# real-stanford/garmentnets

Measured on AMD Instinct MI355X. Metric: garments/s end-to-end predict (PointNet++ -> gridding -> UNet3D -> WNF decode -> marching cubes), higher is better.
Workload: dtype f32 (f16x2 convs, f16x2 decoder MLPs, fp32 accumulation)

## Files before the change

### garmentnets_amd/_lib.py

```python
import ctypes
import os

_HERE = os.path.dirname(os.path.abspath(__file__))
LIB_PATH = os.environ.get("GARMENTNETS_HIP_LIB") or os.path.join(_HERE, "libgarmentnets_hip.so")

GN_OK, GN_EINVAL, GN_ELAUNCH, GN_ECAP = 0, -1, -2, -3

_vp, _i32, _i64, _f32, _f64, _sz = (ctypes.c_void_p, ctypes.c_int, ctypes.c_int64, ctypes.c_float, ctypes.c_double,
                                   ctypes.c_size_t)

PROTOTYPES = {
    "gn_version": [],
    "gn_device_info": [_vp, _vp],
    "gn_segment_ptr": [_vp, _i64, _i32, _vp, _vp],
    "gn_fps": [_vp, _vp, _vp, _vp, _i32, _i32, _vp, _vp],
    "gn_fps_nested": [_vp, _vp, _vp, _vp, _i32, _i32, _vp, _vp, _vp, _vp],
    "gn_fps_workspace_bytes": [_i32, _i32],
    "gn_fps_nested_ws": [_vp, _vp, _vp, _vp, _i32, _i32, _vp, _vp, _vp, _vp, _sz, _vp],
    "gn_ball_query": [_vp, _vp, _vp, _vp, _i32, _i32, _f32, _i32, _vp, _vp, _vp],
    "gn_sa_gather": [_vp, _i32, _i32, _vp, _vp, _vp, _i32, _i32, _i32, _vp, _i32, _vp, _vp],
    "gn_segment_max": [_vp, _i32, _vp, _i32, _i32, _i32, _vp, _i32, _vp],
    "gn_sa_fused_supported": [_i32, _i32, _i32, _i32],
    "gn_sa_fused": [_vp, _i32, _i32, _vp, _vp, _vp, _vp, _i32, _i32, _i32, _vp, _vp, _vp, _vp, _i32, _i32, _i32, _vp, _i32, _vp],
    "gn_sa_fused_scoped": [_vp, _i32, _i32, _vp, _vp, _vp, _vp, _i32, _i32, _i32, _vp, _vp, _vp, _vp, _vp, _i32, _i32, _i32, _vp, _i32, _vp],
    "gn_sa_fused_group": [_vp, _i32, _i32, _vp, _vp, _vp, _vp, _i32, _i32, _i32, _vp, _vp, _vp, _vp, _vp, _i32, _i32, _i32, _vp, _i32, _vp, _i32],
    "gn_sa_fused_auto_group": [_i32, _i32, _i32, _i32, _i32],
    "gn_sa_gather_scoped": [_vp, _i32, _i32, _vp, _vp, _vp, _i32, _i32, _i32, _vp, _vp, _i32, _vp, _vp],
    "gn_global_max_pool": [_vp, _i32, _vp, _i32, _i32, _vp, _i32, _vp],
    "gn_knn_interpolate": [_vp, _i32, _vp, _vp, _vp, _vp, _i32, _i32, _i32, _i32, _vp, _i32, _vp],
    "gn_knn_interpolate_any": [_vp, _i32, _vp, _vp, _vp, _vp, _i32, _i32, _i32, _i32, _vp, _i32, _vp],
    "gn_linear": [_vp, _i32, _vp, _i32, _vp, _vp, _vp, _i32, _i64, _i32, _i32, _vp, _i32, _vp],
    "gn_nocs_head": [_vp, _i32, _i64, _i32, _vp, _vp, _vp, _vp],
    "gn_grid_features": [_vp, _i32, _i32, _vp, _vp, _vp, _vp, _i64, _vp, _vp, _vp, _i32, _i32, _vp, _i32, _vp, _vp],
    "gn_grid_scatter_workspace_bytes": [_i64, _i32, _i32],
    "gn_grid_scatter": [_vp, _i32, _vp, _i64, _i32, _i64, _i32, _vp, _vp, _vp, _sz, _i32, _vp],
    "gn_grid_scatter_ex": [_vp, _i32, _vp, _i64, _i32, _i32, _i64, _i32, _vp, _vp, _vp, _sz, _i32, _vp],
    "gn_channel_stats": [_vp, _i32, _i64, _i32, _vp, _vp, _vp],
    "gn_groupnorm_affine": [_vp, _vp, _i32, _i64, _vp, _vp, _i32, _i64, _i32, _i32, _i32, _f32, _vp, _vp, _vp, _vp, _vp, _vp],
    "gn_channel_stats_any": [_vp, _i32, _i64, _i32, _vp, _vp, _vp],
    "gn_groupnorm_affine_map": [_vp, _vp, _i32, _i32, _i64, _vp, _vp, _i32, _i32, _i64, _i32, _i32, _i32, _f32, _vp, _vp, _vp, _vp, _vp, _vp],
    "gn_conv3d_gcr": [_vp, _i32, _vp, _i32, _vp, _vp, _vp, _i32, _i32, _i32, _i32, _i32, _i32, _vp, _vp, _vp, _vp],
    "gn_conv3d_gcr_split": [_vp, _i32, _vp, _i32, _vp, _vp, _vp, _i32, _vp, _vp, _i32, _i32, _i32, _i32, _i32, _i32, _vp, _vp, _vp, _vp, _vp, _i32, _vp, _vp, _sz, _vp],
    "gn_conv3d_occupancy_workspace_bytes": [_i32, _i32, _i32, _i32],
    "gn_conv_affine_pack_bytes": [_i32, _i32, _i32],
    "gn_conv_affine_pack": [_vp, _i32, _i32, _vp, _vp, _vp, _vp, _i64, _vp, _i32, _vp, _sz, _vp, _vp, _vp, _vp, _vp, _sz, _vp],
    "gn_conv3d_gcr_split_persample": [_vp, _i32, _vp, _vp, _vp, _vp, _vp, _i32, _i32, _i32, _i32, _i32, _i32, _vp, _vp, _vp, _vp, _vp, _i32, _vp, _vp, _sz, _vp],
    "gn_conv_affine_pack_wino_bytes": [_i32, _i32, _i32],
    "gn_conv_affine_pack_wino": [_vp, _i32, _i32, _vp, _vp, _vp, _vp, _i64, _vp, _i32, _vp, _sz, _vp, _vp, _vp, _vp, _vp, _sz, _vp],
    "gn_conv3d_gcr_split_wino": [_vp, _i32, _vp, _vp, _vp, _vp, _vp, _vp, _i32, _i32, _i32, _i32, _i32, _i32, _vp, _vp, _vp, _vp, _vp, _i32, _vp, _sz, _vp],
    "gn_conv3d_gcr_split_wino_partial": [_vp, _i32, _vp, _vp, _vp, _vp, _vp, _vp, _i32, _i32, _i32, _i32, _i32, _i32, _vp, _vp, _vp, _vp, _vp],
    "gn_weight_pack_split_bytes": [_i32, _i32, _i32],
    "gn_weight_pack_split_wino_bytes": [_i32, _i32],
    "gn_weight_pack_upconv_bytes": [_i32, _i32],
    "gn_weight_pack_split": [_vp, _i32, _i32, _i32, _i32, _i32, _vp, _sz, _vp, _vp],
    "gn_weight_pack_split_wino": [_vp, _i32, _i32, _i32, _i32, _vp, _sz, _vp, _vp],
    "gn_weight_pack_upconv": [_vp, _i32, _i32, _i32, _i32, _vp, _sz, _vp, _vp],
    "gn_affine_act": [_vp, _i32, _i64, _i32, _vp, _vp, _vp, _i32, _vp, _vp],
    "gn_upconv_partial": [_vp, _i32, _vp, _vp, _vp, _i32, _vp, _vp, _i32, _i32, _i32, _i32, _i32, _vp, _vp],
    "gn_grid_tile_flags": [_vp, _i64, _i32, _i32, _i32, _i32, _i32, _vp, _vp],
    "gn_maxpool3d_2": [_vp, _i32, _i32, _i32, _i32, _i32, _vp, _vp, _vp, _vp],
    "gn_grid_stats": [_vp, _vp, _i64, _i32, _i64, _i32, _vp, _vp, _vp, _vp],
    "gn_trilinear_sample": [_vp, _i32, _i32, _i32, _i32, _vp, _i32, _i64, _i64, _vp, _i32, _vp],
    "gn_trilinear_sample_batch": [_vp, _i32, _i64, _i32, _i32, _i32, _i32, _vp, _i64, _vp, _i32, _vp],
    "gn_implicit_decode": [_vp, _i32, _i32, _i32, _i32, _vp, _i32, _vp, _i32, _i64, _i64, _vp, _vp, _vp, _vp, _i32, _vp, _vp, _vp, _vp, _i32,
                           _vp, _vp, _vp, _vp, _i32, _vp, _i32, _vp, _vp],
    "gn_ggm3d": [_vp, _i32, _i32, _i32, _f64, _vp, _vp, _vp],
    "gn_minmax": [_vp, _i64, _vp, _vp],
    "gn_ggm3d_batch": [_vp, _i32, _i32, _i32, _i32, _f64, _vp, _vp, _vp],
    "gn_ggm3d_range_workspace_bytes": [_i32, _i32, _i32, _i32],
    "gn_ggm3d_batch_ex": [_vp, _i32, _i32, _i32, _i32, _f64, _vp, _vp, _i32, _vp, _vp, _sz, _vp],
    "gn_minmax_batch": [_vp, _i32, _i64, _vp, _vp],
    "gn_mc33_batch_workspace_bytes": [_i32, _i32, _i32, _i32],
    "gn_mc33_batch": [_vp, _i32, _i32, _i32, _i32, _f64, _vp, _sz, _vp, _vp, _vp, _vp, _i64, _i64, _vp, _vp],
    "gn_mc33_batch_profiled": [_vp, _i32, _i32, _i32, _i32, _f64, _vp, _sz, _vp, _vp, _vp, _vp, _i64, _i64, _vp, _vp, _vp],
    "gn_mc33_workspace_bytes": [_i32, _i32, _i32],
    "gn_mc33": [_vp, _i32, _i32, _i32, _f64, _vp, _sz, _vp, _vp, _vp, _vp, _i64, _i64, _vp, _vp],
    "gn_gather_nn": [_vp, _i32, _i32, _i32, _vp, _i64, _f64, _vp, _vp],
    "gn_gather_nn_batch": [_vp, _i32, _i32, _i32, _i32, _vp, _i64, _f64, _vp, _vp],
    "gn_mesh_compact_workspace_bytes": [_i64, _i64],
    "gn_mesh_largest_component_workspace_bytes": [_i64],
    "gn_mesh_largest_component": [_vp, _i64, _i64, _vp, _sz, _vp, _vp, _vp, _vp],
    "gn_mesh_compact": [_vp, _i32, _vp, _vp, _i64, _i64, _vp, _sz, _vp, _vp, _vp, _vp],
    "gn_scale_verts": [_vp, _i64, _f64, _vp, _vp],
    "gn_implicit_decode_split": [_vp, _i32, _i64, _vp, _vp, _vp, _i32, _i32, _i32, _i32, _vp, _i32, _vp],
    "gn_implicit_decode_split_batch": [_vp, _i32, _i64, _i32, _vp, _vp, _vp, _i32, _i32, _i32, _i32, _vp, _i32, _vp],
    "gn_implicit_decode_batch": [_vp, _i32, _i64, _i32, _i32, _vp, _vp, _vp, _vp, _i32, _vp, _vp, _vp, _vp, _i32, _vp, _vp, _vp, _vp, _i32, _vp, _i32, _vp, _i32, _vp],
    "gn_implicit_decode_lattice_split": [_vp, _i32, _i32, _i32, _i32, _i32, _i64, _i64, _vp, _vp, _vp, _i32, _i32, _i32, _vp, _i32, _vp],
    "gn_decoder_input_scale": [_vp, _i64, _i32, _i32, _f32, _vp, _vp],
    "gn_nearest_neighbor": [_vp, _i64, _vp, _i64, _vp, _vp, _vp],
    "gn_nearest_neighbor_f64_batch": [_vp, _vp, _vp, _i32, _i64, _vp, _vp, _vp],
    "gn_point_mesh_sqdist_batch": [_vp, _vp, _vp, _vp, _i32, _i64, _vp, _vp, _vp, _vp],
    "gn_winding_number_batch": [_vp, _vp, _vp, _vp, _i32, _i64, _vp, _vp, _vp],
    "gn_winding_field_batch": [_vp, _vp, _vp, _i32, _i32, _i32, _i32, _vp, _vp, _vp],
    "gn_distance_field_batch": [_vp, _vp, _vp, _i32, _i32, _i32, _i32, _vp, _vp, _vp, _vp],
    "gn_query_targets_face_chunk": [],
    "gn_query_targets_workspace_bytes": [_i32, _i64, _i64, _i32],
    "gn_query_targets_batch": [_vp, _vp, _vp, _vp, _i32, _i64, _i64, _i32, _i32, _f32, _i32, _vp, _sz, _vp, _vp, _vp, _vp, _vp, _vp],
    "gn_nocs_bin_metrics_workspace_bytes": [_vp, _i32],
    "gn_nocs_bin_metrics": [_vp, _i32, _i32, _i32, _vp, _sz, _vp, _vp],
    "gn_value_losses_workspace_bytes": [_vp, _i32],
    "gn_value_losses": [_vp, _i32, _vp, _sz, _vp, _vp],
    "gn_nocs_bin_loss_bwd": [_vp, _i32, _i32, _i32, _vp, _vp, _vp, _vp],
    "gn_value_losses_bwd": [_vp, _i32, _vp, _vp, _vp],
    "gn_adam_step": [_vp, _i32, _i64, _vp, _i32, _vp],
    "gn_grad_pack": [_vp, _i32, _i64, _vp, _i64, _i32, _vp],
    "gn_grid_scatter_bwd_workspace_bytes": [_i64, _i32, _i64, _i32],
    "gn_grid_scatter_bwd": [_vp, _vp, _vp, _i32, _vp, _i64, _i32, _i32, _i64, _i32, _vp, _sz, _vp, _i32, _vp],
    "gn_segment_max_bwd": [_vp, _i32, _vp, _i32, _vp, _i32, _vp, _i32, _i32, _i32, _vp, _i32, _vp],
    "gn_global_max_pool_bwd": [_vp, _i32, _vp, _i32, _vp, _i32, _vp, _i32, _i32, _vp, _i32, _vp],
    "gn_sa_gather_bwd_workspace_bytes": [_i64, _i64],
    "gn_sa_gather_bwd": [_vp, _i32, _vp, _i64, _i32, _i64, _vp, _sz, _vp, _i32, _vp],
    "gn_knn_neighbours": [_vp, _vp, _vp, _vp, _i32, _i32, _i32, _vp, _vp, _vp],
    "gn_knn_interpolate_bwd_workspace_bytes": [_i64, _i32, _i64],
    "gn_knn_interpolate_bwd": [_vp, _vp, _i32, _i32, _vp, _i32, _i32, _i32, _vp, _sz, _vp, _i32, _vp],
    "gn_trilinear_sample_bwd_workspace_bytes": [_i32, _i64, _i32, _i32, _i32],
    "gn_trilinear_sample_bwd": [_vp, _i32, _vp, _i32, _i32, _i32, _i32, _i32, _vp, _i64, _vp, _sz, _vp, _vp, _vp],
    "gn_conv3d_bwd_weight_workspace_bytes": [_i32, _i32, _i32, _i32, _i32, _i32],
    "gn_conv3d_bwd_weight": [_vp, _i32, _vp, _i32, _vp, _vp, _vp, _vp, _i32, _i32, _i32, _i32, _i32, _vp, _sz, _vp, _vp],
    "gn_relu_mask": [_vp, _vp, _i64, _vp, _vp],
    "gn_relu_mask_max_workspace_bytes": [_i32],
    "gn_relu_mask_max": [_vp, _vp, _i32, _i64, _i32, _vp, _vp, _vp, _vp, _vp, _sz, _vp],
    "gn_conv3d_bwd_weight_split_workspace_bytes": [_i32, _i32, _i32, _i32, _i32, _i32],
    "gn_conv3d_bwd_weight_split": [_vp, _i32, _vp, _i32, _vp, _vp, _vp, _vp, _vp, _vp, _i32, _i32, _i32, _i32, _i32, _vp, _sz, _vp, _vp],
    "gn_groupnorm_bwd_stats_workspace_bytes": [_i32, _i64, _i32],
    "gn_groupnorm_bwd_stats": [_vp, _i32, _i32, _vp, _i32, _i32, _i32, _i32, _i32, _i32, _vp, _sz, _vp, _vp, _vp],
    "gn_groupnorm_bwd_coef": [_vp, _vp, _vp, _vp, _i32, _i32, _i64, _vp, _vp, _vp, _vp, _i32, _i32, _i64, _i32, _i32, _i32, _f32, _vp, _vp, _vp, _vp, _vp,
                              _vp, _vp],
    "gn_groupnorm_bwd_apply": [_vp, _i32, _i32, _vp, _i32, _i32, _i32, _i32, _i32, _i32, _vp, _vp, _vp, _i32, _i32, _i32, _vp, _vp],
    "gn_maxpool3d_2_bwd": [_vp, _vp, _i32, _i32, _i32, _i32, _i32, _vp, _vp],
    "gn_linear_act_bwd_workspace_bytes": [_i64, _i32],
    "gn_linear_act_bwd": [_vp, _i32, _vp, _i32, _vp, _i64, _i32, _vp, _i32, _vp, _sz, _vp, _vp],
    "gn_linear_bwd_weight_workspace_bytes": [_i64, _i32, _i32],
    "gn_linear_bwd_weight": [_vp, _i32, _vp, _i32, _i64, _i32, _i32, _vp, _sz, _vp, _i32, _vp],
    "gn_row_affine": [_vp, _i32, _vp, _vp, _i64, _i32, _vp, _i32, _vp],
    "gn_col_moments_workspace_bytes": [_i64, _i32],
    "gn_col_moments": [_vp, _i32, _i64, _i32, _vp, _sz, _vp, _vp],
    "gn_col_dots_workspace_bytes": [_i64, _i32],
    "gn_col_dots": [_vp, _i32, _vp, _i32, _i64, _i32, _vp, _sz, _vp, _vp],
    "gn_bn_train_bwd_workspace_bytes": [_i64, _i32],
    "gn_bn_train_bwd": [_vp, _i32, _vp, _i32, _vp, _i64, _i32, _vp, _i32, _vp, _sz, _vp, _vp],
    "gn_resident_points": [_vp, _vp, _i32, _i32, _vp, _vp, _vp, _vp, _vp, _vp, _vp, _vp],
    "gn_resident_garment": [_vp, _vp, _i32, _i32, _vp, _vp, _vp, _vp, _vp, _vp, _vp, _vp, _vp, _vp],
    "gn_resident_volume": [_vp, _vp, _i32, _i32, _i32, _vp, _vp, _vp, _vp, _vp, _i32, _vp, _vp, _vp],
    "gn_resident_volume_queries": [_vp, _vp, _i32, _i32, _i32, _vp, _vp, _vp, _vp, _vp, _vp, _vp, _vp],
    "gn_resident_query_targets": [_vp, _vp, _i32, _i64, _i32, _i64, _i64, _i32, _i32, _f32, _i32, _vp, _vp, _sz, _vp, _vp, _vp],
    "gn_resident_surface": [_vp, _vp, _i32, _i32, _vp, _vp, _i32, _vp, _vp, _vp, _vp],
    "gn_resident_mc_surface": [_vp, _vp, _i32, _i32, _vp, _vp, _vp, _vp, _vp],
    "gn_render_points_batch": [_vp, _vp, _vp, _vp, _vp, _i32, _i32, _vp, _vp],
    "gn_color_idx_batch": [_vp, _vp, _vp, _vp, _vp, _i32, _i32, _vp, _vp],
    "gn_render_mesh_batch": [_vp, _vp, _vp, _vp, _vp, _vp, _i32, _i32, _vp, _vp],
    "gn_color_mesh_batch": [_vp, _vp, _vp, _vp, _vp, _vp, _vp, _vp, _i32, _i32, _vp, _vp],
    "gn_depth_render_batch": [_vp, _vp, _vp, _vp, _i32, _vp, _vp, _vp, _i32, _i32, _vp, _vp],
    "gn_depth_cloud_offsets": [_vp, _i32, _i32, _vp, _vp, _vp],
    "gn_depth_cloud_write": [_vp, _vp, _vp, _vp, _vp, _vp, _i32, _vp, _vp, _vp, _vp, _i32, _i32, _i64, _vp, _vp, _vp, _vp],
    "gn_cloth_simulate_batch": [_vp, _vp, _vp, _vp, _vp, _vp, _vp, _vp, _i32, _i64, _i64, _i64, _i32, _vp, _i32, _i32, _vp, _vp],
    "gn_cloth_contact_buckets": [_i32],
    "gn_cloth_contact_workspace_bytes": [_i64, _i32, _i32],
    "gn_cloth_contact_lists": [_vp, _vp, _vp, _i32, _i64, _i32, _i32, _vp, _i32, _i32, _vp, _sz, _vp, _vp, _vp, _vp, _vp, _vp],
    "gn_cloth_simulate_contacts_batch": [_vp, _vp, _vp, _vp, _vp, _vp, _vp, _vp, _i32, _i64, _i64, _i64, _i32, _vp, _i32, _i32, _vp, _vp, _vp, _vp,
                                         _i32, _vp, _vp, _vp, _vp],
}
_RESTYPES = {"gn_weight_pack_split_bytes": _sz, "gn_weight_pack_split_wino_bytes": _sz, "gn_weight_pack_upconv_bytes": _sz,
             "gn_conv_affine_pack_bytes": _sz, "gn_conv_affine_pack_wino_bytes": _sz, "gn_conv3d_occupancy_workspace_bytes": _sz, "gn_mc33_workspace_bytes": _sz, "gn_ggm3d_range_workspace_bytes": _sz, "gn_mc33_batch_workspace_bytes": _sz, "gn_grid_scatter_workspace_bytes": _sz, "gn_fps_workspace_bytes": _sz, "gn_mesh_compact_workspace_bytes": _sz, "gn_mesh_largest_component_workspace_bytes": _sz,
             "gn_nocs_bin_metrics_workspace_bytes": _sz, "gn_value_losses_workspace_bytes": _sz,
             "gn_grid_scatter_bwd_workspace_bytes": _sz, "gn_sa_gather_bwd_workspace_bytes": _sz, "gn_knn_interpolate_bwd_workspace_bytes": _sz,
             "gn_trilinear_sample_bwd_workspace_bytes": _sz, "gn_conv3d_bwd_weight_workspace_bytes": _sz, "gn_conv3d_bwd_weight_split_workspace_bytes": _sz, "gn_relu_mask_max_workspace_bytes": _sz, "gn_groupnorm_bwd_stats_workspace_bytes": _sz,
             "gn_linear_act_bwd_workspace_bytes": _sz, "gn_linear_bwd_weight_workspace_bytes": _sz,
             "gn_col_moments_workspace_bytes": _sz, "gn_col_dots_workspace_bytes": _sz, "gn_bn_train_bwd_workspace_bytes": _sz,
             "gn_query_targets_workspace_bytes": _sz, "gn_cloth_contact_workspace_bytes": _sz}

LINEAR_BWD_CHUNK_ROWS = 512
LINEAR_ACT_CHUNK_ROWS = 1024

LOSS_MAX_SETS = 8
LOSS_KINDS = {"l2": 0, "smooth_l1": 1, "bce_logits": 2, "row_norm": 3}


class NocsBinSet(ctypes.Structure):
    _fields_ = [("logits", _vp), ("gt", _vp), ("n", _i64), ("ldl", _i32), ("pad", _i32)]


class LossSegment(ctypes.Structure):
    _fields_ = [("pred", _vp), ("target", _vp), ("count", _i64), ("kind", _i32), ("mirror", _i32)]


class NocsBinGradSet(ctypes.Structure):
    _fields_ = [("logits", _vp), ("gt", _vp), ("grad", _vp), ("n", _i64), ("ldl", _i32), ("ldg", _i32), ("ncols", _i32), ("pad", _i32)]


class LossGradSegment(ctypes.Structure):
    _fields_ = [("pred", _vp), ("target", _vp), ("grad", _vp), ("count", _i64), ("coef", _f64), ("kind", _i32), ("mirror", _i32)]


QT_KINDS = {"nocs_winding_number_field": 0, "sim_nocs_winding_number_field": 0, "nocs_distance_field": 1, "nocs_signed_distance_field": 2,
            "nocs_occupancy_grid": 3}

ADAM_CHUNK = 4096
ADAM_MAX_HYPER = 16


class AdamEntry(ctypes.Structure):
    _fields_ = [("p", _vp), ("g", _vp), ("exp_avg", _vp), ("exp_avg_sq", _vp), ("numel", _i64), ("blk0", _i64), ("hyper", _i32), ("pad", _i32)]


class PackEntry(ctypes.Structure):
    _fields_ = [("src", _vp), ("dst_off", _i64), ("numel", _i64), ("blk0", _i64)]


class AdamHyper(ctypes.Structure):
    _fields_ = [("lr", _f64), ("beta1", _f64), ("beta2", _f64), ("eps", _f64), ("weight_decay", _f64), ("bias_correction1", _f64),
                ("bias_correction2_sqrt", _f64)]


RESIDENT_META = ("pc_off", "pc_len", "vert_off", "face_off", "num_faces", "mc_vert_off", "mc_face_off", "num_mc_faces", "dataset_idx",
                 "scale_bits")
RESIDENT_ARRAYS = ("pc_sim", "pc_nocs", "pc_rgb", "sim_verts", "nocs_verts", "task_verts", "faces", "cdf_nocs", "cdf_task", "mc_verts", "mc_flags",
                   "mc_faces", "cdf_mc", "volume", "meta", "grip", "aabb")


class ResidentStore(ctypes.Structure):
    _fields_ = [(k, _vp) for k in RESIDENT_ARRAYS] + [("n", _i32), ("D", _i32), ("H", _i32), ("W", _i32)]


CLOTH_MAX_LDS = 160 * 1024
CLOTH_MAX_BLOCK = 1024
CLOTH_MAX_LIST = 64
CLOTH_LISTS_TRAVEL, CLOTH_LISTS_BUILD = 1, 2

RENDER_MAX_SIZE = 4096
RENDER_MAX_OVERLAYS = 3
RENDER_SIDES = {"front": 0, "top": 1, "left": 2}
COLOR_TABLE, COLOR_VIRIDIS = 0, 1


class OverlayPoint(ctypes.Structure):
    _fields_ = [("xyz", _f32 * 3), ("rgba", _f32 * 4), ("kernel_size", _i32)]


class ColorImage(ctypes.Structure):
    _fields_ = [("offset", _i64), ("count", _i64), ("mode", _i32), ("side", _i32), ("vmin", _f32), ("vmax", _f32), ("default_color", _f32 * 4),
                ("num_overlays", _i32), ("pad", _i32), ("overlay", OverlayPoint * RENDER_MAX_OVERLAYS)]


class MeshImage(ctypes.Structure):
    _fields_ = [("vert_begin", _i64), ("vert_end", _i64), ("face_begin", _i64), ("face_end", _i64), ("side", _i32), ("ambient", _f32),
                ("default_color", _f32 * 4)]


class DepthImage(ctypes.Structure):
    _fields_ = [("vert_begin", _i64), ("vert_end", _i64), ("face_begin", _i64), ("face_end", _i64), ("R", _f64 * 9), ("t", _f64 * 3), ("f", _f64),
                ("c", _f64), ("znear", _f64), ("ambient", _f32), ("base_color", _f32 * 3)]


_lib = None


class GarmentNetsHipError(RuntimeError):
    pass


def load():
    global _lib
    if _lib is not None:
        return _lib
    if not os.path.exists(LIB_PATH):
        raise GarmentNetsHipError(
            f"{LIB_PATH} not found: build it with `python -c 'import __graft_entry__ as g; g.build()'` "
            "(or `make -C garmentnets_amd/csrc`). garmentnets_amd has no CPU fallback.")
    lib = ctypes.CDLL(LIB_PATH)
    lib.gn_last_error.restype = ctypes.c_char_p
    lib.gn_last_error.argtypes = []
    lib.gn_last_kernel.restype = ctypes.c_char_p
    lib.gn_last_kernel.argtypes = []
    for name, argtypes in PROTOTYPES.items():
        fn = getattr(lib, name)
        fn.argtypes = argtypes
        fn.restype = _RESTYPES.get(name, ctypes.c_int)
    _lib = lib
    return lib


def call(name, *args):
    lib = load()
    rc = getattr(lib, name)(*args)
    if rc != GN_OK:
        msg = lib.gn_last_error().decode(errors="replace")
        if rc == GN_EINVAL:
            raise ValueError(f"{name}: {msg}")
        raise GarmentNetsHipError(f"{name} failed (code {rc}): {msg}")
    return rc
```

### garmentnets_amd/components/pointnet2.py

```python
import os
import threading
import weakref

import numpy as np
import torch

from .. import ops
from .mlp import fold_batchnorm, generation, param_cache

FUSED_SA = os.environ.get("GARMENTNETS_FUSED_SA", "1") != "0"

class _DeviceTableCache:

    def __init__(self, limit=256):
        self._lock, self._tables, self._limit = threading.Lock(), {}, limit

    def get(self, key, build):
        with self._lock:
            t = self._tables.get(key)
            if t is None:
                if len(self._tables) >= self._limit:
                    self._tables.clear()
                t = self._tables[key] = build()
            return t


_DEBUG = threading.local()
_PTR_CACHE = _DeviceTableCache()
_SELF_SRC_CACHE = _DeviceTableCache()


def _csr_ptr(sizes, device):
    return _PTR_CACHE.get((tuple(sizes), str(device)),
                          lambda: torch.tensor(np.concatenate([[0], np.cumsum(sizes)]), dtype=torch.int32).to(device))


def _example_self_src(sizes, centre_sizes, device):
    def build():
        starts = np.concatenate([[0], np.cumsum(sizes)])[:-1]
        return torch.tensor(np.concatenate([s + np.arange(m) for s, m in zip(starts, centre_sizes)] or [np.zeros(0)]), dtype=torch.int32).to(device)
    return _SELF_SRC_CACHE.get((tuple(sizes), tuple(centre_sizes), str(device)), build)


class Segments:

    def __init__(self, sizes, device, batch=None):
        self.sizes = [int(s) for s in sizes]
        self.device = device
        self.ptr = _csr_ptr(self.sizes, device)
        self._batch = batch

    @staticmethod
    def of(batch, sizes=None):
        if isinstance(batch, Segments):
            return batch
        if sizes is None:
            n = int(batch.max().item()) + 1 if batch.numel() else 0
            sizes = torch.bincount(batch, minlength=n).cpu().tolist()
        return Segments(sizes, batch.device, batch)

    @property
    def num(self):
        return len(self.sizes)

    @property
    def total(self):
        return int(sum(self.sizes))

    @property
    def batch(self):
        if self._batch is None:
            self._batch = torch.repeat_interleave(torch.arange(self.num, device=self.device),
                                                  torch.tensor(self.sizes, device=self.device))
        return self._batch


class PointConv(torch.nn.Module):

    def __init__(self, local_nn=None, global_nn=None, add_self_loops=True):
        super().__init__()
        self.local_nn = local_nn
        self.global_nn = global_nn
        self.add_self_loops = add_self_loops
        self.self_loop_scope = "batch"


class SAModule(torch.nn.Module):

    def __init__(self, ratio, r, nn, random_start=False, max_num_neighbors=64):
        super().__init__()
        self.ratio = ratio
        self.r = r
        self.max_num_neighbors = max_num_neighbors
        self.conv = PointConv(nn)
        self.random_start = random_start

    def forward(self, x, pos, batch):
        seg = Segments.of(batch)
        out_sizes = [ops.fps_count(n, self.ratio) for n in seg.sizes]
        cseg = Segments(out_sizes, pos.device)
        start = None
        if self.random_start:
            start = torch.tensor([int(torch.randint(0, max(n, 1), (1,))) for n in seg.sizes], dtype=torch.int32).to(pos.device)
        gap = nested = None
        if start is None and seg.num > 0:
            gap = torch.zeros(seg.num, dtype=torch.float32, device=pos.device)
            src = getattr(pos, "_fps_cascade", None)
            if src is not None and src[1] == seg.sizes and src[2] == pos._version and src[0].device == pos.device:
                nested = src[0]
        idx = ops.fps(pos, seg.ptr, cseg.ptr, max(seg.sizes) if seg.sizes else 0, cseg.total, start, gap_out=gap, nested_gap=nested)
        nbr, cnt = ops.ball_query(pos, seg.ptr, idx, cseg.ptr, self.r, self.max_num_neighbors)
        pack = self._fused_pack() if FUSED_SA else None
        self_src = None
        if self.conv.add_self_loops and self.conv.self_loop_scope == "example" and seg.num > 1:
            self_src = _example_self_src(seg.sizes, out_sizes, pos.device)
        if pack is not None and ((x is None and pack.cin == 0) or (x is not None and x.shape[1] == pack.cin)):
            out = ops.sa_fused(x, pos, idx, nbr, cnt, pack, self_loops=self.conv.add_self_loops, self_src=self_src)
        else:
            edges, slot_src, S = ops.sa_gather(x, pos, idx, nbr, self_loops=self.conv.add_self_loops, self_src=self_src)
            h = self.conv.local_nn(edges)
            out = ops.segment_max(h, slot_src, cseg.total, S)
        _DEBUG.__dict__.setdefault("graphs", weakref.WeakKeyDictionary())[self] = (idx, nbr)
        pos_out = pos[idx.long()]
        if gap is not None:
            pos_out._fps_cascade = (gap, out_sizes, pos_out._version)
        return out, pos_out, cseg

    @property
    def last_graph(self):
        return _DEBUG.__dict__.get("graphs", {}).get(self)

    def _fused_pack(self):
        nn_ = self.conv.local_nn
        blocks = list(nn_) if nn_ is not None else []
        if len(blocks) != 3:
            return None
        dims = [b[0].out_features for b in blocks]
        cin = blocks[0][0].in_features - 3
        if not ops.sa_fused_supported(cin, dims):
            return None
        def build():
            layers = []
            for b in blocks:
                sc, sh = fold_batchnorm(b[2]) if len(b) > 2 else (None, None)
                layers.append((b[0].weight, b[0].bias, sc, sh))
            return ops.pack_sa_fused(layers).to(blocks[0][0].weight.device)
        return param_cache(self, "_sa_pack").get(generation(nn_), "pack", build)


class GlobalSAModule(torch.nn.Module):

    def __init__(self, nn):
        super().__init__()
        self.nn = nn

    def forward(self, x, pos, batch):
        seg = Segments.of(batch)
        c = x.shape[1]
        buf = ops.new_rows(x.shape[0], c + 3, x.device)
        buf[:, :c] = x
        buf[:, c:] = pos
        h = self.nn(buf)
        out = ops.global_max_pool(h, seg.ptr, seg.num)
        return out, pos.new_zeros((seg.num, 3)), Segments([1] * seg.num, pos.device)


class FPModule(torch.nn.Module):

    def __init__(self, k, nn):
        super().__init__()
        self.k = k
        self.nn = nn

    def forward(self, x, pos, batch, x_skip, pos_skip, batch_skip):
        seg, seg_skip = Segments.of(batch), Segments.of(batch_skip)
        c = x.shape[1]
        cs = 0 if x_skip is None else x_skip.shape[1]
        buf = ops.new_rows(pos_skip.shape[0], c + cs, x.device)
        ops.knn_interpolate(x, pos.contiguous(), seg.ptr, pos_skip.contiguous(), seg_skip.ptr, self.k, out=buf[:, :c])
        if x_skip is not None:
            buf[:, c:] = x_skip
        return self.nn(buf), pos_skip, seg_skip
```

### garmentnets_amd/csrc/points.hip

```cpp
#include <stdarg.h>
#include <limits.h>

#include "common.h"

static thread_local char g_err[512] = "";
void gn_set_error(const char *fmt, ...) {
    va_list ap;
    va_start(ap, fmt);
    vsnprintf(g_err, sizeof(g_err), fmt, ap);
    va_end(ap);
}
extern "C" const char *gn_last_error(void) { return g_err; }
extern "C" int gn_version(void) { return 200; }
hipStream_t gn_stream(void *s) {
    hipStream_t st = (hipStream_t)s;
    if (st) {
        hipDevice_t dev = 0;
        int cur = 0;
        if (hipStreamGetDevice(st, &dev) == hipSuccess && hipGetDevice(&cur) == hipSuccess && cur != (int)dev) (void)hipSetDevice((int)dev);
    }
    return st;
}
static thread_local const char *g_last_kernel = "";
void gn_note_kernel(const char *name) { g_last_kernel = name; }
extern "C" const char *gn_last_kernel(void) { return g_last_kernel; }
extern "C" int gn_device_info(int *num_cu, int *lds_bytes_per_cu) {
    int dev = 0;
    hipDeviceProp_t p;
    GN_HIP(hipGetDevice(&dev), "gn_device_info");
    GN_HIP(hipGetDeviceProperties(&p, dev), "gn_device_info");
    if (num_cu) *num_cu = p.multiProcessorCount;
    if (lds_bytes_per_cu) *lds_bytes_per_cu = (int)p.maxSharedMemoryPerMultiProcessor;
    return GN_OK;
}

__global__ void segment_ptr_kernel(const int64_t *__restrict__ batch, int64_t n, int B, int32_t *__restrict__ ptr) {
    int64_t i = (int64_t)blockIdx.x * blockDim.x + threadIdx.x;
    if (i > n) return;
    int64_t lo = (i == 0) ? -1 : batch[i - 1];
    int64_t hi = (i == n) ? (int64_t)B : batch[i];
    if (hi > B) hi = B;
    for (int64_t b = lo + 1; b <= hi; ++b) ptr[b] = (int32_t)i;
}

extern "C" int gn_segment_ptr(const int64_t *batch, int64_t n, int B, int32_t *ptr, void *stream) {
    GN_REQUIRE(n >= 0 && B >= 0 && n < INT32_MAX, "gn_segment_ptr: bad sizes");
    int64_t blocks = gn_cdiv(n + 1, 256);
    hipLaunchKernelGGL(segment_ptr_kernel, dim3((unsigned)blocks), dim3(256), 0, gn_stream(stream), batch, n, B, ptr);
    GN_LAUNCH_CHECK("gn_segment_ptr");
    return GN_OK;
}

#define FPS_THREADS 1024
#define FPS_WAVES (FPS_THREADS / 64)

__device__ __forceinline__ float fps_min(float a, float b) {
    float o;
    asm("v_min_f32 %0, %1, %2" : "=v"(o) : "v"(a), "v"(b));
    return o;
}

template <int WAVES, bool BALLOT>
__device__ __forceinline__ int fps_pick(float bv, int bi, int k, float *pv, int *pi, int lane, int wave, float &gv) {
    const float wv = gn_wave_max(bv);
    int wi;
    if (BALLOT) {
        const unsigned long long hit = __ballot(bv == wv);
        if (__builtin_popcountll(hit) == 1) wi = __builtin_amdgcn_readlane(bi, __builtin_ctzll(hit));
        else wi = gn_wave_min(bv == wv ? bi : INT_MAX);
    } else {
        wi = gn_wave_min(bv == wv ? bi : INT_MAX);
    }
    const int par = (k & 1) * WAVES;
    if (lane == 0) { pv[par + wave] = wv; pi[par + wave] = wi; }
    __syncthreads();
    float fv = pv[par + (lane & (WAVES - 1))];
    int fi = pi[par + (lane & (WAVES - 1))];
    gv = gn_row_max<WAVES>(fv);
    fi = gn_row_min<WAVES>(fv == gv ? fi : INT_MAX);
    return __builtin_amdgcn_readfirstlane(fi);
}

template <int PPT, bool LDS_POS, int THREADS>
__global__ __launch_bounds__(THREADS) void fps_kernel(const float *__restrict__ pos, const int32_t *__restrict__ ptr,
                                                      const int32_t *__restrict__ out_ptr, const int32_t *__restrict__ start_idx,
                                                      int32_t *__restrict__ out_idx, float *__restrict__ gap_out,
                                                      const float *__restrict__ nested_gap) {
    constexpr int WAVES = THREADS / 64;
    static_assert(PPT == 1 || PPT % 2 == 0, "points are updated in pairs");
    extern __shared__ __attribute__((aligned(16))) float smem[];
    const int b = blockIdx.x;
    const int s = ptr[b], n = ptr[b + 1] - s;
    const int o0 = out_ptr[b], m = out_ptr[b + 1] - o0;
    if (n <= 0 || m <= 0) return;
    const int tid = threadIdx.x, lane = tid & 63, wave = tid >> 6;
    if (nested_gap && nested_gap[b] > 0.f && m <= n) {
        for (int k = tid; k < m; k += THREADS) out_idx[o0 + k] = s + k;
        if (gap_out && tid == 0) gap_out[b] = nested_gap[b];
        return;
    }
    float gmin = 3.0e38f;
    float *pv = smem;
    int *pi = (int *)(smem + 2 * WAVES);
    float *lx = smem + 4 * WAVES;
    float *ly = lx + n, *lz = ly + n;
    const float *gp = pos + 3 * (size_t)s;

    float px[PPT], py[PPT], pz[PPT], dd[PPT];
#pragma unroll
    for (int j = 0; j < PPT; ++j) {
        int i = tid + j * THREADS;
        if (i < n) {
            px[j] = gp[3 * i]; py[j] = gp[3 * i + 1]; pz[j] = gp[3 * i + 2];
            if (LDS_POS) { lx[i] = px[j]; ly[i] = py[j]; lz[i] = pz[j]; }
            dd[j] = 3.0e38f;
        } else {
            px[j] = py[j] = pz[j] = 0.f;
            dd[j] = -1.f;
        }
    }
    if (LDS_POS) __syncthreads();
    int last = start_idx ? start_idx[b] : 0;
    if (last < 0 || last >= n) last = 0;
    if (tid == 0) out_idx[o0] = s + last;
    for (int k = 1; k < m; ++k) {
        float qx, qy, qz;
        if (LDS_POS) { qx = lx[last]; qy = ly[last]; qz = lz[last]; }
        else { qx = gp[3 * last]; qy = gp[3 * last + 1]; qz = gp[3 * last + 2]; }
        float bv = -1.f;
        int bj = 0;
        if (PPT == 1) {
            const float d = fps_min(dd[0], gn_sqdist3(px[0], py[0], pz[0], qx, qy, qz));
            dd[0] = d;
            bv = d > bv ? d : bv;
        } else {
            const f32x2 q2x = {qx, qx}, q2y = {qy, qy}, q2z = {qz, qz};
#pragma unroll
            for (int j = 0; j < PPT; j += 2) {
                const f32x2 dx = (f32x2){px[j], px[j + 1]} - q2x, dy = (f32x2){py[j], py[j + 1]} - q2y, dz = (f32x2){pz[j], pz[j + 1]} - q2z;
                const f32x2 d2 = (dx * dx + dy * dy) + dz * dz;
#pragma unroll
                for (int u = 0; u < 2; ++u) {
                    const float d = fps_min(dd[j + u], u ? d2.y : d2.x);
                    dd[j + u] = d;
                    if (d > bv) { bv = d; bj = j + u; }
                }
            }
        }
        const int bi = bv >= 0.f ? tid + bj * THREADS : INT_MAX;
        float gv;
        last = fps_pick<WAVES, true>(bv, bi, k, pv, pi, lane, wave, gv);
        gmin = fps_min(gmin, gv);
        if (tid == 0) out_idx[o0 + k] = s + last;
    }
    if (gap_out && tid == 0) gap_out[b] = gmin;
}

#define FPS_LDS_MAX (36 * 1024)
template <bool IN_WS>
__global__ __launch_bounds__(FPS_THREADS) void fps_large_kernel(const float *__restrict__ pos, const int32_t *__restrict__ ptr, const int32_t *__restrict__ out_ptr,
                                                               const int32_t *__restrict__ start_idx, int32_t *__restrict__ out_idx, float *__restrict__ gap_out,
                                                               const float *__restrict__ nested_gap, float4 *__restrict__ ws, int max_points) {
    constexpr int WAVES = FPS_WAVES;
    extern __shared__ __attribute__((aligned(16))) float smem[];
    const int b = blockIdx.x;
    const int s = ptr[b], n = ptr[b + 1] - s;
    const int o0 = out_ptr[b], m = out_ptr[b + 1] - o0;
    if (n <= 0 || m <= 0) return;
    if (IN_WS && n > max_points) return;
    const int tid = threadIdx.x, lane = tid & 63, wave = tid >> 6;
    if (nested_gap && nested_gap[b] > 0.f && m <= n) {
        for (int k = tid; k < m; k += FPS_THREADS) out_idx[o0 + k] = s + k;
        if (gap_out && tid == 0) gap_out[b] = nested_gap[b];
        return;
    }
    float *pv = smem;
    int *pi = (int *)(smem + 2 * WAVES);
    float *dd = smem + 4 * WAVES;
    float4 *rec = IN_WS ? ws + (size_t)b * max_points : nullptr;
    const float *gp = pos + 3 * (size_t)s;
    for (int i = tid; i < n; i += FPS_THREADS) {
        if (IN_WS) rec[i] = make_float4(gp[3 * i], gp[3 * i + 1], gp[3 * i + 2], 3.0e38f);
        else dd[i] = 3.0e38f;
    }
    if (!IN_WS) __syncthreads();
    float gmin = 3.0e38f;
    int last = start_idx ? start_idx[b] : 0;
    if (last < 0 || last >= n) last = 0;
    if (tid == 0) out_idx[o0] = s + last;
    for (int k = 1; k < m; ++k) {
        const float qx = gp[3 * last], qy = gp[3 * last + 1], qz = gp[3 * last + 2];
        float bv = -1.f;
        int bi = INT_MAX;
        for (int i = tid; i < n; i += FPS_THREADS) {
            float d;
            if (IN_WS) {
                const float4 r = rec[i];
                d = fps_min(r.w, gn_sqdist3(r.x, r.y, r.z, qx, qy, qz));
                reinterpret_cast<float *>(rec + i)[3] = d;
            } else {
                d = fps_min(dd[i], gn_sqdist3(gp[3 * i], gp[3 * i + 1], gp[3 * i + 2], qx, qy, qz));
                dd[i] = d;
            }
            if (d > bv) { bv = d; bi = i; }
        }
        float gv;
        last = fps_pick<WAVES, false>(bv, bi, k, pv, pi, lane, wave, gv);
        gmin = fps_min(gmin, gv);
        if (tid == 0) out_idx[o0 + k] = s + last;
    }
    if (gap_out && tid == 0) gap_out[b] = gmin;
}

extern "C" size_t gn_fps_workspace_bytes(int B, int max_points_per_example) {
    if (B <= 0 || max_points_per_example <= FPS_LDS_MAX) return 0;
    return (size_t)B * (size_t)max_points_per_example * sizeof(float4);
}

static int fps_checked_launch(const float *pos, const int32_t *ptr, const int32_t *out_ptr, const int32_t *start_idx, int B, int n, int32_t *out_idx,
                              float *gap_out, const float *nested_gap, bool takes_ws, void *ws, size_t ws_bytes, void *stream) {
    GN_REQUIRE(B >= 0 && n >= 0, "gn_fps: bad sizes");
    GN_REQUIRE(nested_gap == nullptr || start_idx == nullptr, "gn_fps_nested: a nested sample starts at the example's first point (start_idx must be NULL)");
    if (B == 0 || n == 0) return GN_OK;
    if (n > FPS_LDS_MAX) {
        GN_REQUIRE(takes_ws, "gn_fps: more than %d points per example needs a workspace: gn_fps_nested_ws (got %d)", FPS_LDS_MAX, n);
        const size_t need = gn_fps_workspace_bytes(B, n);
        GN_REQUIRE(ws != nullptr && ws_bytes >= need, "gn_fps_nested_ws: %d points per example need a workspace of %zu bytes (gn_fps_workspace_bytes), got %zu",
                   n, need, ws ? ws_bytes : (size_t)0);
        GN_REQUIRE(((uintptr_t)ws & 15) == 0, "gn_fps_nested_ws: the workspace must be 16-byte aligned");
        hipLaunchKernelGGL(fps_large_kernel<true>, dim3(B), dim3(FPS_THREADS), sizeof(float) * 4 * FPS_WAVES, gn_stream(stream), pos, ptr, out_ptr, start_idx,
                           out_idx, gap_out, nested_gap, reinterpret_cast<float4 *>(ws), n);
        GN_LAUNCH_CHECK("gn_fps");
        return GN_OK;
    }
    if (n > 16 * FPS_THREADS) {
        const size_t shl = sizeof(float) * (4 * FPS_WAVES + (size_t)n);
        GN_HIP(hipFuncSetAttribute((const void *)fps_large_kernel<false>, hipFuncAttributeMaxDynamicSharedMemorySize, (int)shl), "gn_fps");
        hipLaunchKernelGGL(fps_large_kernel<false>, dim3(B), dim3(FPS_THREADS), shl, gn_stream(stream), pos, ptr, out_ptr, start_idx, out_idx, gap_out,
                           nested_gap, (float4 *)nullptr, 0);
        GN_LAUNCH_CHECK("gn_fps");
        return GN_OK;
    }
    const bool lds_pos = n <= 8192;
#ifndef FPS_MID_THREADS
#define FPS_MID_THREADS 512
#endif
    const int threads = n <= 24 * 256 ? 256 : (n <= 24 * FPS_MID_THREADS ? FPS_MID_THREADS : FPS_THREADS);
    size_t sh = sizeof(float) * 4 * (threads / 64) + (lds_pos ? sizeof(float) * 3 * (size_t)n : 0);
    const int ppt = (int)gn_cdiv(n, threads);
#define FPS_LAUNCH(P, L, T)                                                                                     \
    do {                                                                                                        \
        GN_HIP(hipFuncSetAttribute((const void *)fps_kernel<P, L, T>, hipFuncAttributeMaxDynamicSharedMemorySize, (int)sh), "gn_fps"); \
        hipLaunchKernelGGL((fps_kernel<P, L, T>), dim3(B), dim3(T), sh, gn_stream(stream), pos, ptr, out_ptr, start_idx, out_idx, gap_out, nested_gap); \
    } while (0)
#define FPS_BY_PPT(L, T)                               \
    do {                                               \
        if (ppt <= 2) FPS_LAUNCH(2, L, T);             \
        else if (ppt <= 4) FPS_LAUNCH(4, L, T);        \
        else if (ppt <= 6) FPS_LAUNCH(6, L, T);        \
        else if (ppt <= 8) FPS_LAUNCH(8, L, T);        \
        else if (ppt <= 12) FPS_LAUNCH(12, L, T);      \
        else if (ppt <= 16) FPS_LAUNCH(16, L, T);      \
        else FPS_LAUNCH(24, L, T);                     \
    } while (0)
    if (threads == 256) FPS_BY_PPT(true, 256);
    else if (threads == FPS_MID_THREADS && lds_pos) FPS_BY_PPT(true, FPS_MID_THREADS);
    else if (threads == FPS_MID_THREADS) FPS_BY_PPT(false, FPS_MID_THREADS);
    else FPS_LAUNCH(16, false, FPS_THREADS);
#undef FPS_BY_PPT
#undef FPS_LAUNCH
    GN_LAUNCH_CHECK("gn_fps");
    return GN_OK;
}

extern "C" int gn_fps(const float *pos, const int32_t *ptr, const int32_t *out_ptr, const int32_t *start_idx, int B,
                      int max_points_per_example, int32_t *out_idx, void *stream) {
    return fps_checked_launch(pos, ptr, out_ptr, start_idx, B, max_points_per_example, out_idx, nullptr, nullptr, false, nullptr, 0, stream);
}

extern "C" int gn_fps_nested(const float *pos, const int32_t *ptr, const int32_t *out_ptr, const int32_t *start_idx, int B,
                             int max_points_per_example, int32_t *out_idx, float *gap_out, const float *nested_gap, void *stream) {
    return fps_checked_launch(pos, ptr, out_ptr, start_idx, B, max_points_per_example, out_idx, gap_out, nested_gap, false, nullptr, 0, stream);
}

extern "C" int gn_fps_nested_ws(const float *pos, const int32_t *ptr, const int32_t *out_ptr, const int32_t *start_idx, int B,
                                int max_points_per_example, int32_t *out_idx, float *gap_out, const float *nested_gap, void *ws, size_t ws_bytes,
                                void *stream) {
    return fps_checked_launch(pos, ptr, out_ptr, start_idx, B, max_points_per_example, out_idx, gap_out, nested_gap, true, ws, ws_bytes, stream);
}

__global__ __launch_bounds__(256) void ball_query_kernel(const float *__restrict__ pos, const int32_t *__restrict__ ptr,
                                                         const int32_t *__restrict__ centre_idx,
                                                         const int32_t *__restrict__ centre_ptr, int B, int M, float r2, int K,
                                                         int32_t *__restrict__ nbr, int32_t *__restrict__ cnt) {
    const int lane = threadIdx.x & 63;
    const int c = blockIdx.x * (blockDim.x >> 6) + (threadIdx.x >> 6);
    if (c >= M) return;
    int lo = 0, hi = B;
    while (hi - lo > 1) {
        int mid = (lo + hi) >> 1;
        if (centre_ptr[mid] <= c) lo = mid; else hi = mid;
    }
    const int b = lo;
    const int s = ptr[b], e = ptr[b + 1];
    const int ci = centre_idx[c];
    const float cx = pos[3 * (size_t)ci], cy = pos[3 * (size_t)ci + 1], cz = pos[3 * (size_t)ci + 2];
    int32_t *row = nbr + (size_t)c * K;
    int count = 0;
    for (int base = s; base < e && count < K; base += 64) {
        int j = base + lane;
        bool in = false;
        if (j < e) {
            float d = gn_sqdist3(pos[3 * (size_t)j], pos[3 * (size_t)j + 1], pos[3 * (size_t)j + 2], cx, cy, cz);
            in = d < r2;
        }
        unsigned long long mask = __ballot(in);
        int before = __popcll(mask & ((1ull << lane) - 1ull));
        if (in && count + before < K) row[count + before] = j;
        count += __popcll(mask);
    }
    if (count > K) count = K;
    for (int t = count + lane; t < K; t += 64) row[t] = -1;
    if (lane == 0) cnt[c] = count;
}

extern "C" int gn_ball_query(const float *pos, const int32_t *ptr, const int32_t *centre_idx, const int32_t *centre_ptr,
                             int B, int M, float r2, int K, int32_t *nbr, int32_t *cnt, void *stream) {
    GN_REQUIRE(B >= 0 && M >= 0 && K > 0, "gn_ball_query: bad sizes");
    if (M == 0) return GN_OK;
    hipLaunchKernelGGL(ball_query_kernel, dim3((unsigned)gn_cdiv(M, 4)), dim3(256), 0, gn_stream(stream), pos, ptr, centre_idx,
                       centre_ptr, B, M, r2, K, nbr, cnt);
    GN_LAUNCH_CHECK("gn_ball_query");
    return GN_OK;
}

__global__ __launch_bounds__(256) void sa_gather_kernel(const float *__restrict__ x, int ldx, int C, const float *__restrict__ pos,
                                                        const int32_t *__restrict__ centre_idx, const int32_t *__restrict__ nbr,
                                                        int M, int K, int self_loops, const int32_t *__restrict__ self_src,
                                                        float *__restrict__ out, int ldo, int32_t *__restrict__ slot_src) {
    const int lane = threadIdx.x & 63;
    const int64_t row = (int64_t)blockIdx.x * (blockDim.x >> 6) + (threadIdx.x >> 6);
    const int S = K + (self_loops ? 1 : 0);
    if (row >= (int64_t)M * S) return;
    const int c = (int)(row / S), sl = (int)(row % S);
    const int self = self_src ? self_src[c] : c;
    int j;
    if (sl < K) {
        j = nbr[(size_t)c * K + sl];
        if (self_loops && j == self) j = -1;
    } else {
        j = self;
    }
    float *o = out + row * (int64_t)ldo;
    if (lane == 0) slot_src[row] = j;
    if (j < 0) {
        for (int t = lane; t < C + 3; t += 64) o[t] = 0.f;
        return;
    }
    const float *xr = x ? x + (size_t)j * ldx : nullptr;
    for (int t = lane; t < C; t += 64) o[t] = xr[t];
    if (lane < 3) {
        int ci = centre_idx[c];
        o[C + lane] = __fsub_rn(pos[3 * (size_t)j + lane], pos[3 * (size_t)ci + lane]);
    }
}

extern "C" int gn_sa_gather_scoped(const float *x, int ldx, int C, const float *pos, const int32_t *centre_idx, const int32_t *nbr,
                                   int M, int K, int self_loops, const int32_t *self_src, float *out, int ldo, int32_t *slot_src,
                                   void *stream) {
    GN_REQUIRE(M >= 0 && K > 0 && C >= 0 && ldo >= C + 3, "gn_sa_gather: bad sizes");
    GN_REQUIRE(C == 0 || x != nullptr, "gn_sa_gather: x is NULL with C>0");
    if (M == 0) return GN_OK;
    int64_t rows = (int64_t)M * (K + (self_loops ? 1 : 0));
    hipLaunchKernelGGL(sa_gather_kernel, dim3((unsigned)gn_cdiv(rows, 4)), dim3(256), 0, gn_stream(stream), x, ldx, C, pos,
                       centre_idx, nbr, M, K, self_loops, self_src, out, ldo, slot_src);
    GN_LAUNCH_CHECK("gn_sa_gather");
    return GN_OK;
}

extern "C" int gn_sa_gather(const float *x, int ldx, int C, const float *pos, const int32_t *centre_idx, const int32_t *nbr,
                            int M, int K, int self_loops, float *out, int ldo, int32_t *slot_src, void *stream) {
    return gn_sa_gather_scoped(x, ldx, C, pos, centre_idx, nbr, M, K, self_loops, nullptr, out, ldo, slot_src, stream);
}

__global__ __launch_bounds__(256) void segment_max_kernel(const float *__restrict__ in, int ldi, const int32_t *__restrict__ slot_src,
                                                          int M, int S, int C, float *__restrict__ out, int ldo) {
    const int c = blockIdx.x;
    for (int ch = threadIdx.x; ch < C; ch += blockDim.x) {
        float v = 0.f;
        bool any = false;
        for (int s = 0; s < S; ++s) {
            int64_t row = (int64_t)c * S + s;
            if (slot_src[row] < 0) continue;
            float t = in[row * ldi + ch];
            v = any ? fmaxf(v, t) : t;
            any = true;
        }
        out[(int64_t)c * ldo + ch] = v;
    }
}

extern "C" int gn_segment_max(const float *in, int ldi, const int32_t *slot_src, int M, int S, int C, float *out, int ldo,
                              void *stream) {
    GN_REQUIRE(M >= 0 && S > 0 && C > 0, "gn_segment_max: bad sizes");
    if (M == 0) return GN_OK;
    int threads = C >= 256 ? 256 : (C >= 128 ? 128 : 64);
    hipLaunchKernelGGL(segment_max_kernel, dim3(M), dim3(threads), 0, gn_stream(stream), in, ldi, slot_src, M, S, C, out, ldo);
    GN_LAUNCH_CHECK("gn_segment_max");
    return GN_OK;
}

#define GMAX_GROUPS 16
__global__ __launch_bounds__(64 * GMAX_GROUPS) void global_max_kernel(const float *__restrict__ in, int ldi, const int32_t *__restrict__ ptr,
                                                                     int C, float *__restrict__ out, int ldo) {
    __shared__ float part[GMAX_GROUPS][64];
    const int b = blockIdx.x, ch = blockIdx.y * 64 + (threadIdx.x & 63), g = threadIdx.x >> 6;
    const int s = ptr[b], e = ptr[b + 1];
    float v = -3.4e38f;
    if (ch < C)
        for (int r = s + g; r < e; r += GMAX_GROUPS) v = fmaxf(v, in[(int64_t)r * ldi + ch]);
    part[g][threadIdx.x & 63] = v;
    __syncthreads();
    if (g == 0 && ch < C) {
#pragma unroll
        for (int k = 1; k < GMAX_GROUPS; ++k) v = fmaxf(v, part[k][threadIdx.x]);
        out[(int64_t)b * ldo + ch] = (e > s) ? v : 0.f;
    }
}

extern "C" int gn_global_max_pool(const float *in, int ldi, const int32_t *ptr, int B, int C, float *out, int ldo, void *stream) {
    GN_REQUIRE(B >= 0 && C > 0, "gn_global_max_pool: bad sizes");
    if (B == 0) return GN_OK;
    hipLaunchKernelGGL(global_max_kernel, dim3(B, (unsigned)gn_cdiv(C, 64)), dim3(64 * GMAX_GROUPS), 0, gn_stream(stream), in, ldi, ptr, C, out, ldo);
    GN_LAUNCH_CHECK("gn_global_max_pool");
    return GN_OK;
}

#define KNN_MAXK 8
template <int KK>
__global__ __launch_bounds__(256) void knn_interp_kernel(const float *__restrict__ xs, int ldx, const float *__restrict__ ps,
                                                         const int32_t *__restrict__ ptr_s, const float *__restrict__ pq,
                                                         const int32_t *__restrict__ ptr_q, int B, int Nq, int C,
                                                         float *__restrict__ out, int ldo) {
    const int lane = threadIdx.x & 63;
    const int q = blockIdx.x * (blockDim.x >> 6) + (threadIdx.x >> 6);
    if (q >= Nq) return;
    int lo = 0, hi = B;
    while (hi - lo > 1) {
        int mid = (lo + hi) >> 1;
        if (ptr_q[mid] <= q) lo = mid; else hi = mid;
    }
    const int s = ptr_s[lo], e = ptr_s[lo + 1];
    const float qx = pq[3 * (size_t)q], qy = pq[3 * (size_t)q + 1], qz = pq[3 * (size_t)q + 2];
    float bd[KK];
    int bi[KK];
#pragma unroll
    for (int t = 0; t < KK; ++t) { bd[t] = 3.4e38f; bi[t] = INT_MAX; }
    for (int j = s + lane; j < e; j += 64) {
        float d = gn_sqdist3(ps[3 * (size_t)j], ps[3 * (size_t)j + 1], ps[3 * (size_t)j + 2], qx, qy, qz);
        if (d < bd[KK - 1]) {
            bd[KK - 1] = d; bi[KK - 1] = j;
#pragma unroll
            for (int t = KK - 1; t > 0; --t) {
                if (bd[t] < bd[t - 1]) {
                    float td = bd[t]; bd[t] = bd[t - 1]; bd[t - 1] = td;
                    int ti = bi[t]; bi[t] = bi[t - 1]; bi[t - 1] = ti;
                }
            }
        }
    }
    float wd[KK];
    int wi[KK];
    int nsel = 0;
#pragma unroll
    for (int r = 0; r < KK; ++r) {
        float v = bd[0];
        int i = bi[0];
        GN_WAVE_ARGMIN(v, i)
        wd[r] = v; wi[r] = i;
        if (i != INT_MAX) nsel = r + 1;
        if (bi[0] == i && i != INT_MAX) {
#pragma unroll
            for (int t = 0; t < KK - 1; ++t) { bd[t] = bd[t + 1]; bi[t] = bi[t + 1]; }
            bd[KK - 1] = 3.4e38f; bi[KK - 1] = INT_MAX;
        }
    }
    float w[KK];
    float wsum = 0.f;
#pragma unroll
    for (int r = 0; r < KK; ++r) {
        if (r < nsel) {
            float d = wd[r] < 1e-16f ? 1e-16f : wd[r];
            w[r] = __fdiv_rn(1.0f, d);
            wsum = __fadd_rn(wsum, w[r]);
        } else w[r] = 0.f;
    }
    for (int ch = lane; ch < C; ch += 64) {
        float acc = 0.f;
#pragma unroll
        for (int r = 0; r < KK; ++r)
            if (r < nsel) acc = __fadd_rn(acc, __fmul_rn(xs[(size_t)wi[r] * ldx + ch], w[r]));
        out[(size_t)q * ldo + ch] = __fdiv_rn(acc, wsum);
    }
}

extern "C" int gn_knn_interpolate(const float *xs, int ldx, const float *ps, const int32_t *ptr_s, const float *pq,
                                  const int32_t *ptr_q, int B, int Nq, int C, int k, float *out, int ldo, void *stream) {
    GN_REQUIRE(k >= 1 && k <= KNN_MAXK, "gn_knn_interpolate: k must be in [1,%d] (gn_knn_interpolate_any takes any k)", KNN_MAXK);
    GN_REQUIRE(B >= 0 && Nq >= 0 && C > 0, "gn_knn_interpolate: bad sizes");
    if (Nq == 0) return GN_OK;
    dim3 grid((unsigned)gn_cdiv(Nq, 4)), block(256);
#define KNN_LAUNCH(KK) hipLaunchKernelGGL((knn_interp_kernel<KK>), grid, block, 0, gn_stream(stream), xs, ldx, ps, ptr_s, pq, ptr_q, B, Nq, C, out, ldo)
    switch (k) {
        case 1: KNN_LAUNCH(1); break;
        case 2: KNN_LAUNCH(2); break;
        case 3: KNN_LAUNCH(3); break;
        case 4: KNN_LAUNCH(4); break;
        case 5: KNN_LAUNCH(5); break;
        case 6: KNN_LAUNCH(6); break;
        case 7: KNN_LAUNCH(7); break;
        default: KNN_LAUNCH(8); break;
    }
#undef KNN_LAUNCH
    GN_LAUNCH_CHECK("gn_knn_interpolate");
    return GN_OK;
}

__global__ __launch_bounds__(256) void knn_interp_any_kernel(const float *__restrict__ xs, int ldx, const float *__restrict__ ps,
                                                             const int32_t *__restrict__ ptr_s, const float *__restrict__ pq,
                                                             const int32_t *__restrict__ ptr_q, int B, int Nq, int C, int k,
                                                             float *__restrict__ out, int ldo) {
    const int lane = threadIdx.x & 63;
    const int q = blockIdx.x * (blockDim.x >> 6) + (threadIdx.x >> 6);
    if (q >= Nq) return;
    int lo = 0, hi = B;
    while (hi - lo > 1) {
        int mid = (lo + hi) >> 1;
        if (ptr_q[mid] <= q) lo = mid; else hi = mid;
    }
    const int s = ptr_s[lo], e = ptr_s[lo + 1];
    const float qx = pq[3 * (size_t)q], qy = pq[3 * (size_t)q + 1], qz = pq[3 * (size_t)q + 2];
    float *o = out + (size_t)q * ldo;
    for (int ch = lane; ch < C; ch += 64) o[ch] = 0.f;
    float pd = -1.f;
    int pj = -1;
    float wsum = 0.f;
    for (int r = 0; r < k; ++r) {
        float v = 3.4e38f;
        int i = INT_MAX;
        for (int j = s + lane; j < e; j += 64) {
            const float d = gn_sqdist3(ps[3 * (size_t)j], ps[3 * (size_t)j + 1], ps[3 * (size_t)j + 2], qx, qy, qz);
            if ((d > pd || (d == pd && j > pj)) && d < v) { v = d; i = j; }
        }
        GN_WAVE_ARGMIN(v, i)
        if (i == INT_MAX) break;
        pd = v;
        pj = i;
        const float w = __fdiv_rn(1.0f, v < 1e-16f ? 1e-16f : v);
        wsum = __fadd_rn(wsum, w);
        const float *xr = xs + (size_t)i * ldx;
        for (int ch = lane; ch < C; ch += 64) o[ch] = __fadd_rn(o[ch], __fmul_rn(xr[ch], w));
    }
    for (int ch = lane; ch < C; ch += 64) o[ch] = __fdiv_rn(o[ch], wsum);
}

extern "C" int gn_knn_interpolate_any(const float *xs, int ldx, const float *ps, const int32_t *ptr_s, const float *pq,
                                      const int32_t *ptr_q, int B, int Nq, int C, int k, float *out, int ldo, void *stream) {
    GN_REQUIRE(k >= 1, "gn_knn_interpolate_any: k must be >= 1");
    GN_REQUIRE(B >= 0 && Nq >= 0 && C > 0, "gn_knn_interpolate_any: bad sizes");
    if (Nq == 0) return GN_OK;
    if (k <= KNN_MAXK) return gn_knn_interpolate(xs, ldx, ps, ptr_s, pq, ptr_q, B, Nq, C, k, out, ldo, stream);
    hipLaunchKernelGGL(knn_interp_any_kernel, dim3((unsigned)gn_cdiv(Nq, 4)), dim3(256), 0, gn_stream(stream), xs, ldx, ps, ptr_s, pq, ptr_q, B, Nq, C, k,
                       out, ldo);
    GN_LAUNCH_CHECK("gn_knn_interpolate_any");
    return GN_OK;
}

__global__ __launch_bounds__(256) void nocs_head_kernel(const float *__restrict__ logits, int ldl, int64_t N, int bins,
                                                        int64_t *__restrict__ bin_idx, float *__restrict__ conf,
                                                        float *__restrict__ nocs) {
    int64_t t = (int64_t)blockIdx.x * blockDim.x + threadIdx.x;
    if (t >= N * 3) return;
    int64_t p = t / 3;
    int a = (int)(t % 3);
    const float *row = logits + p * ldl;
    float mx = row[a];
    int arg = 0;
    for (int k = 1; k < bins; ++k) {
        float v = row[k * 3 + a];
        if (v > mx) { mx = v; arg = k; }
    }
    float sum = 0.f;
    for (int k = 0; k < bins; ++k) sum = __fadd_rn(sum, expf(__fsub_rn(row[k * 3 + a], mx)));
    bin_idx[t] = arg;
    conf[t] = __fdiv_rn(1.0f, sum);
    const float scale = __fdiv_rn(1.0f, __fsub_rn((float)bins, 1.0f));
    nocs[t] = __fadd_rn(__fmul_rn((float)arg, scale), 0.0f);
}

extern "C" int gn_nocs_head(const float *logits, int ldl, int64_t N, int bins, int64_t *bin_idx, float *confidence,
                            float *pred_nocs, void *stream) {
    GN_REQUIRE(N >= 0 && bins > 0 && ldl >= bins * 3, "gn_nocs_head: bad sizes");
    if (N == 0) return GN_OK;
    hipLaunchKernelGGL(nocs_head_kernel, dim3((unsigned)gn_cdiv(N * 3, 256)), dim3(256), 0, gn_stream(stream), logits, ldl, N, bins,
                       bin_idx, confidence, pred_nocs);
    GN_LAUNCH_CHECK("gn_nocs_head");
    return GN_OK;
}

#define NN_TILE 1024
__global__ __launch_bounds__(256) void nearest_neighbor_kernel(const float *__restrict__ q, int64_t nq, const float *__restrict__ ref,
                                                               int64_t nr, int32_t *__restrict__ idx, float *__restrict__ d2) {
    __shared__ float sx[NN_TILE], sy[NN_TILE], sz[NN_TILE];
    const int64_t i = (int64_t)blockIdx.x * blockDim.x + threadIdx.x;
    float qx = 0.f, qy = 0.f, qz = 0.f;
    if (i < nq) { qx = q[3 * i]; qy = q[3 * i + 1]; qz = q[3 * i + 2]; }
    float best = 3.4e38f;
    int bi = -1;
    for (int64_t t0 = 0; t0 < nr; t0 += NN_TILE) {
        const int n = (int)((nr - t0) < NN_TILE ? (nr - t0) : NN_TILE);
        __syncthreads();
        for (int j = threadIdx.x; j < n; j += blockDim.x) { sx[j] = ref[3 * (t0 + j)]; sy[j] = ref[3 * (t0 + j) + 1]; sz[j] = ref[3 * (t0 + j) + 2]; }
        __syncthreads();
        for (int j = 0; j < n; ++j) {
            const float d = gn_sqdist3(sx[j], sy[j], sz[j], qx, qy, qz);
            if (d < best) { best = d; bi = (int)(t0 + j); }
        }
    }
    if (i < nq) { idx[i] = bi; d2[i] = best; }
}

extern "C" int gn_nearest_neighbor(const float *query, int64_t nq, const float *ref, int64_t nr, int32_t *idx, float *d2, void *stream) {
    GN_REQUIRE(nq >= 0 && nr > 0 && nr < INT32_MAX, "gn_nearest_neighbor: bad sizes (the reference set must not be empty)");
    if (nq == 0) return GN_OK;
    hipLaunchKernelGGL(nearest_neighbor_kernel, dim3((unsigned)gn_cdiv(nq, 256)), dim3(256), 0, gn_stream(stream), query, nq, ref, nr, idx, d2);
// ... 4 lines not shown
```

### garmentnets_amd/csrc/sa_fused.hip

```cpp
#include "common.h"

struct SaArgs {
    const float *x; int ldx;
    const float *pos;
    const int32_t *centre_idx;
    const int32_t *nbr;
    const int32_t *cnt;
    int M, K, self_loops;
    const int32_t *self_src;
    const float4 *w1, *w2, *w3;
    const float *tab;
    float *out; int ldo;
};

__device__ __forceinline__ f32x16 sa_mfma(float a, float b, const f32x16 &c) { return __builtin_amdgcn_mfma_f32_32x32x2f32(a, b, c, 0, 0, 0); }

__device__ __forceinline__ void sa_epilogue(f32x16 &a, const float *tb) {
#pragma unroll
    for (int q4 = 0; q4 < 4; ++q4) {
        const float4 b = *reinterpret_cast<const float4 *>(tb + 4 * q4);
        const float4 sc = *reinterpret_cast<const float4 *>(tb + 16 + 4 * q4);
        const float4 sh = *reinterpret_cast<const float4 *>(tb + 32 + 4 * q4);
        a[4 * q4 + 0] = __fadd_rn(__fmul_rn(gn_relu(__fadd_rn(a[4 * q4 + 0], b.x)), sc.x), sh.x);
        a[4 * q4 + 1] = __fadd_rn(__fmul_rn(gn_relu(__fadd_rn(a[4 * q4 + 1], b.y)), sc.y), sh.y);
        a[4 * q4 + 2] = __fadd_rn(__fmul_rn(gn_relu(__fadd_rn(a[4 * q4 + 2], b.z)), sc.z), sh.z);
        a[4 * q4 + 3] = __fadd_rn(__fmul_rn(gn_relu(__fadd_rn(a[4 * q4 + 3], b.w)), sc.w), sh.w);
    }
}

template <int NKB, int LASTQ, typename BF>
__device__ __forceinline__ void sa_block(f32x16 &acc, const float4 *&w, BF bsrc) {
    float4 wc[4], wn[4];
#pragma unroll
    for (int qq = 0; qq < 4; ++qq) wc[qq] = w[qq * 64];
#pragma unroll
    for (int kb = 0; kb < NKB; ++kb) {
        if (kb + 1 < NKB) {
#pragma unroll
            for (int qq = 0; qq < 4; ++qq) wn[qq] = w[256 + qq * 64];
        }
#pragma unroll
        for (int qq = 0; qq < 4; ++qq) {
            if (kb == NKB - 1 && qq >= LASTQ) continue;
            acc = sa_mfma(wc[qq].x, bsrc(kb, 4 * qq + 0), acc);
            acc = sa_mfma(wc[qq].y, bsrc(kb, 4 * qq + 1), acc);
            acc = sa_mfma(wc[qq].z, bsrc(kb, 4 * qq + 2), acc);
            acc = sa_mfma(wc[qq].w, bsrc(kb, 4 * qq + 3), acc);
        }
        __builtin_amdgcn_sched_barrier(0);
#pragma unroll
        for (int qq = 0; qq < 4; ++qq) wc[qq] = wn[qq];
        w += 256;
    }
}

template <int CIN, int N1, int N2, int N3, int G>
__global__ __launch_bounds__(256, 2) void sa_fused_kernel(SaArgs p) {
    constexpr int K1 = CIN + 3, K1P = (K1 + 7) & ~7, KB1 = (K1P + 31) / 32;
    constexpr int LASTQ1 = (K1P - 32 * (KB1 - 1)) / 8;
    constexpr int NB1 = N1 / 32, NB2 = N2 / 32, NB3 = N3 / 32;
    constexpr int TAB2 = NB1 * 96, TAB3 = TAB2 + NB2 * 96, TABN = TAB3 + NB3 * 96;
    static_assert(N1 % 32 == 0 && N2 % 32 == 0 && N3 % 32 == 0 && G <= 32, "block sizes");
    __shared__ int out_lds[G * N3];
    __shared__ __attribute__((aligned(16))) float tab[TABN];
    __shared__ int tile_ctr;
    const int tid = threadIdx.x, lane = tid & 63, h = lane >> 5, r = lane & 31;
    const int c0 = blockIdx.x * G;
    for (int i = tid; i < G * N3; i += 256) out_lds[i] = gn_sord_enc(-INFINITY);
    for (int i = tid; i < TABN; i += 256) tab[i] = p.tab[i];
    if (tid == 0) tile_ctr = 0;
    __syncthreads();
    const int ntiles = 2 * G + (p.self_loops ? 1 : 0);

    for (;;) {
        int t = 0;
        if (lane == 0) t = atomicAdd(&tile_ctr, 1);
        t = __builtin_amdgcn_readfirstlane(t);
        if (t >= ntiles) break;
        int j, ci, cl;
        if (t < 2 * G) {
            cl = t >> 1;
            const int c = c0 + cl, half = t & 1;
            if (c >= p.M) continue;
            if (p.cnt[c] <= 32 * half) continue;
            const int slot = 32 * half + r;
            j = slot < p.K ? p.nbr[(size_t)c * p.K + slot] : -1;
            if (p.self_loops && j == (p.self_src ? p.self_src[c] : c)) j = -1;
            ci = p.centre_idx[c];
        } else {
            const int c = c0 + r;
            const bool ok = r < G && c < p.M;
            cl = r;
            j = ok ? (p.self_src ? p.self_src[c] : c) : -1;
            ci = ok ? p.centre_idx[c] : 0;
        }
        const bool valid = j >= 0;
        const size_t jj = valid ? (size_t)j : 0;
        const float r0 = __fsub_rn(p.pos[3 * jj + 0], p.pos[3 * (size_t)ci + 0]);
        const float r1 = __fsub_rn(p.pos[3 * jj + 1], p.pos[3 * (size_t)ci + 1]);
        const float r2 = __fsub_rn(p.pos[3 * jj + 2], p.pos[3 * (size_t)ci + 2]);
        const float *xr = CIN > 0 ? p.x + jj * p.ldx : nullptr;

        float xin[KB1 * 16];
#pragma unroll
        for (int kb = 0; kb < KB1; ++kb)
#pragma unroll
            for (int qq = 0; qq < 4; ++qq) {
                const int kk = 32 * kb + 8 * qq;
                if (kk + 8 <= CIN) {
                    const float4 v = *reinterpret_cast<const float4 *>(xr + kk + 4 * h);
                    xin[16 * kb + 4 * qq + 0] = v.x; xin[16 * kb + 4 * qq + 1] = v.y; xin[16 * kb + 4 * qq + 2] = v.z; xin[16 * kb + 4 * qq + 3] = v.w;
                } else {
#pragma unroll
                    for (int i = 0; i < 4; ++i) {
                        const int k = kk + 4 * h + i, rk = k - CIN;
                        float v = 0.f;
                        if (kk < K1P) {
                            if (k < CIN) v = xr[k];
                            else if (rk == 0) v = r0;
                            else if (rk == 1) v = r1;
                            else if (rk == 2) v = r2;
                        }
                        xin[16 * kb + 4 * qq + i] = v;
                    }
                }
            }

        const float4 *w1 = p.w1 + lane, *w2 = p.w2 + lane, *w3 = p.w3 + lane;
        asm volatile("" : "+v"(w1), "+v"(w2), "+v"(w3));
        f32x16 a1[NB1];
#pragma unroll
        for (int nb = 0; nb < NB1; ++nb) {
#pragma unroll
            for (int q = 0; q < 16; ++q) a1[nb][q] = 0.f;
            sa_block<KB1, LASTQ1>(a1[nb], w1, [&](int kb, int q) { return xin[16 * kb + q]; });
            sa_epilogue(a1[nb], tab + (nb * 2 + h) * 48);
        }
        f32x16 a2[NB2];
#pragma unroll
        for (int nb = 0; nb < NB2; ++nb) {
#pragma unroll
            for (int q = 0; q < 16; ++q) a2[nb][q] = 0.f;
            sa_block<NB1, 4>(a2[nb], w2, [&](int kb, int q) { return a1[kb][q]; });
            sa_epilogue(a2[nb], tab + TAB2 + (nb * 2 + h) * 48);
        }
        const bool self_tile = t >= 2 * G;
#pragma unroll 1
        for (int nb = 0; nb < NB3; ++nb) {
            f32x16 a3;
#pragma unroll
            for (int q = 0; q < 16; ++q) a3[q] = 0.f;
            sa_block<NB2, 4>(a3, w3, [&](int kb, int q) { return a2[kb][q]; });
            sa_epilogue(a3, tab + TAB3 + (nb * 2 + h) * 48);
            int *const o = out_lds + cl * N3 + 32 * nb + 4 * h;
            if (self_tile) {
                if (valid) {
#pragma unroll
                    for (int q = 0; q < 16; ++q) atomicMax(o + 8 * (q >> 2) + (q & 3), gn_sord_enc(a3[q]));
                }
            } else {
#pragma unroll
                for (int q = 0; q < 16; ++q) {
                    const float m = gn_half_max(valid ? a3[q] : -INFINITY);
                    if (r == 0) atomicMax(o + 8 * (q >> 2) + (q & 3), gn_sord_enc(m));
                }
            }
        }
    }
    __syncthreads();
    for (int i = tid; i < G * N3; i += 256) {
        const int cl = i / N3, u = i % N3, c = c0 + cl;
        if (c < p.M) {
            const float v = gn_sord_dec(out_lds[i]);
            p.out[(size_t)c * p.ldo + u] = v == -INFINITY ? 0.f : v;
        }
    }
}

template <int CIN, int N1, int N2, int N3, int G>
static int sa_slots() {
    static const int slots = [] {
        int per_cu = 0, dev = 0, cus = 256;
        if (hipOccupancyMaxActiveBlocksPerMultiprocessor(&per_cu, (const void *)sa_fused_kernel<CIN, N1, N2, N3, G>, 256, 0) != hipSuccess || per_cu < 1) per_cu = 2;
        hipDeviceProp_t pr;
        if (hipGetDevice(&dev) == hipSuccess && hipGetDeviceProperties(&pr, dev) == hipSuccess && pr.multiProcessorCount > 0) cus = pr.multiProcessorCount;
        return per_cu * cus;
    }();
    return slots;
}
template <int CIN, int N1, int N2, int N3, int G>
static double sa_cost(int M) {
    const double n = (double)gn_cdiv(M, G), slots = (double)sa_slots<CIN, N1, N2, N3, G>();
    const double rounds = (double)gn_cdiv((int64_t)n, (int64_t)slots);
    return (2.0 * G + 1.0) / (2.0 * G) * rounds * slots / n;
}
template <int CIN, int N1, int N2, int N3>
static int sa_auto_group(int M) {
    const double c32 = sa_cost<CIN, N1, N2, N3, 32>(M), c16 = sa_cost<CIN, N1, N2, N3, 16>(M), c8 = sa_cost<CIN, N1, N2, N3, 8>(M),
                 c4 = sa_cost<CIN, N1, N2, N3, 4>(M), c2 = sa_cost<CIN, N1, N2, N3, 2>(M);
    double best = c32;
    int g = 32;
    if (c16 < best) { best = c16; g = 16; }
    if (c8 < best) { best = c8; g = 8; }
    if (c4 < best) { best = c4; g = 4; }
    if (c2 < best) { best = c2; g = 2; }
    return g;
}
template <int CIN, int N1, int N2, int N3>
static int sa_launch(const SaArgs &p, hipStream_t st, int group) {
    switch (group ? group : sa_auto_group<CIN, N1, N2, N3>(p.M)) {
        case 32: hipLaunchKernelGGL((sa_fused_kernel<CIN, N1, N2, N3, 32>), dim3((unsigned)gn_cdiv(p.M, 32)), dim3(256), 0, st, p); break;
        case 16: hipLaunchKernelGGL((sa_fused_kernel<CIN, N1, N2, N3, 16>), dim3((unsigned)gn_cdiv(p.M, 16)), dim3(256), 0, st, p); break;
        case 8: hipLaunchKernelGGL((sa_fused_kernel<CIN, N1, N2, N3, 8>), dim3((unsigned)gn_cdiv(p.M, 8)), dim3(256), 0, st, p); break;
        case 4: hipLaunchKernelGGL((sa_fused_kernel<CIN, N1, N2, N3, 4>), dim3((unsigned)gn_cdiv(p.M, 4)), dim3(256), 0, st, p); break;
        default: hipLaunchKernelGGL((sa_fused_kernel<CIN, N1, N2, N3, 2>), dim3((unsigned)gn_cdiv(p.M, 2)), dim3(256), 0, st, p); break;
    }
    return 0;
}

#define SA_SHAPES(X)                                                                                                           \
    X(3, 64, 64, 128) X(128, 128, 128, 256)                                                                                    \
    X(3, 32, 32, 64) X(3, 32, 64, 128) X(3, 64, 64, 64) X(3, 64, 128, 128)                                                     \
    X(64, 64, 64, 128) X(64, 64, 128, 256) X(128, 128, 128, 128) X(128, 128, 256, 256) X(0, 64, 64, 128)

extern "C" int gn_sa_fused_supported(int C, int N1, int N2, int N3) {
#define SA_MATCH(c, n1, n2, n3) if (C == c && N1 == n1 && N2 == n2 && N3 == n3) return 1;
    SA_SHAPES(SA_MATCH)
#undef SA_MATCH
    return 0;
}

extern "C" int gn_sa_fused_auto_group(int C, int N1, int N2, int N3, int M) {
    GN_REQUIRE(M >= 0, "gn_sa_fused_auto_group: bad sizes");
    GN_REQUIRE(gn_sa_fused_supported(C, N1, N2, N3), "gn_sa_fused_auto_group: edge MLP [%d+3,%d,%d,%d] is not instantiated (see SA_SHAPES in csrc/sa_fused.hip)", C, N1, N2, N3);
#define SA_AUTO(c, n1, n2, n3) if (C == c && N1 == n1 && N2 == n2 && N3 == n3) return sa_auto_group<c, n1, n2, n3>(M);
    SA_SHAPES(SA_AUTO)
#undef SA_AUTO
    return GN_EINVAL;
}

extern "C" int gn_sa_fused_group(const float *x, int ldx, int C, const float *pos, const int32_t *centre_idx, const int32_t *nbr,
                                 const int32_t *cnt, int M, int K, int self_loops, const int32_t *self_src, const float *w1p,
                                 const float *w2p, const float *w3p, const float *tab, int N1, int N2, int N3, float *out, int ldo,
                                 void *stream, int group) {
    GN_REQUIRE(M >= 0 && K > 0 && K <= 64 && ldo >= N3, "gn_sa_fused: bad sizes (the ball-query table holds at most 64 neighbours)");
    GN_REQUIRE(group == 0 || group == 2 || group == 4 || group == 8 || group == 16 || group == 32, "gn_sa_fused: group %d is not one of 0 (the cost rule), 2, 4, 8, 16, 32", group);
    GN_REQUIRE(gn_sa_fused_supported(C, N1, N2, N3), "gn_sa_fused: edge MLP [%d+3,%d,%d,%d] is not instantiated (see SA_SHAPES in csrc/sa_fused.hip); use gn_sa_gather + gn_linear + gn_segment_max", C, N1, N2, N3);
    GN_REQUIRE(C == 0 || (x && ldx >= C && (C < 8 || (ldx % 4 == 0 && (uintptr_t)x % 16 == 0))), "gn_sa_fused: feature rows need a 16-byte aligned base and leading dimension");
    if (M == 0) return GN_OK;
    GN_REQUIRE(pos && centre_idx && nbr && cnt && w1p && w2p && w3p && tab && out, "gn_sa_fused: null pointer");
    SaArgs p;
    p.x = x; p.ldx = ldx; p.pos = pos; p.centre_idx = centre_idx; p.nbr = nbr; p.cnt = cnt; p.M = M; p.K = K; p.self_loops = self_loops;
    p.self_src = self_src;
    p.w1 = (const float4 *)w1p; p.w2 = (const float4 *)w2p; p.w3 = (const float4 *)w3p; p.tab = tab; p.out = out; p.ldo = ldo;
    hipStream_t st = gn_stream(stream);
#define SA_DISPATCH(c, n1, n2, n3) if (C == c && N1 == n1 && N2 == n2 && N3 == n3) sa_launch<c, n1, n2, n3>(p, st, group);
    SA_SHAPES(SA_DISPATCH)
#undef SA_DISPATCH
    GN_LAUNCH_CHECK("gn_sa_fused");
    return GN_OK;
}

extern "C" int gn_sa_fused_scoped(const float *x, int ldx, int C, const float *pos, const int32_t *centre_idx, const int32_t *nbr,
                                  const int32_t *cnt, int M, int K, int self_loops, const int32_t *self_src, const float *w1p,
                                  const float *w2p, const float *w3p, const float *tab, int N1, int N2, int N3, float *out, int ldo,
                                  void *stream) {
    return gn_sa_fused_group(x, ldx, C, pos, centre_idx, nbr, cnt, M, K, self_loops, self_src, w1p, w2p, w3p, tab, N1, N2, N3, out, ldo, stream, 0);
}

extern "C" int gn_sa_fused(const float *x, int ldx, int C, const float *pos, const int32_t *centre_idx, const int32_t *nbr, const int32_t *cnt,
                           int M, int K, int self_loops, const float *w1p, const float *w2p, const float *w3p, const float *tab, int N1, int N2,
                           int N3, float *out, int ldo, void *stream) {
    return gn_sa_fused_group(x, ldx, C, pos, centre_idx, nbr, cnt, M, K, self_loops, nullptr, w1p, w2p, w3p, tab, N1, N2, N3, out, ldo, stream, 0);
}
```

### garmentnets_amd/ops.py

```python
import ctypes
import math
import threading

import numpy as np
import torch

from . import _lib

_i32 = torch.int32


class _CallState(threading.local):
    dev = None


_CALL = _CallState()


def _stream():
    dev, _CALL.dev = _CALL.dev, None
    if dev is not None and dev.index is not None and dev.index != torch.cuda.current_device():
        torch.cuda.set_device(dev)
    return ctypes.c_void_p(torch.cuda.current_stream(dev).cuda_stream)


def _p(t):
    if t is None:
        return None
    if not t.is_cuda:
        raise _lib.GarmentNetsHipError("garmentnets_amd ops need tensors on the GPU (no CPU fallback)")
    if _CALL.dev is None:
        _CALL.dev = t.device
    elif _CALL.dev != t.device:
        dev, _CALL.dev = _CALL.dev, None
        raise _lib.GarmentNetsHipError(f"garmentnets_amd ops: tensors on different devices ({dev} vs {t.device})")
    return ctypes.c_void_p(t.data_ptr())


def _chk(t, dtype, name):
    if t.dtype != dtype:
        raise TypeError(f"{name}: expected {dtype}, got {t.dtype}")
    if not t.is_contiguous():
        raise ValueError(f"{name}: tensor must be contiguous")
    return t


def pad4(c):
    return (c + 3) // 4 * 4


def rows_view(t):
    assert t.dim() == 2 and (t.shape[1] == 1 or t.stride(1) == 1), "need row-major rows"
    return t.shape[0], (t.stride(0) if t.shape[0] > 1 else max(t.stride(0), t.shape[1]))


def new_rows(n, c, device):
    buf = torch.empty((n, pad4(c)), dtype=torch.float32, device=device)
    return buf[:, :c]


def fps_count(n, ratio):
    return int(math.ceil(float(np.float32(n) * np.float32(ratio))))


def segment_ptr(batch, B):
    _chk(batch, torch.int64, "batch")
    ptr = torch.empty(B + 1, dtype=_i32, device=batch.device)
    _lib.call("gn_segment_ptr", _p(batch), batch.numel(), B, _p(ptr), _stream())
    return ptr


def fps(pos, ptr, out_ptr, max_points, m_total, start_idx=None, gap_out=None, nested_gap=None):
    _chk(pos, torch.float32, "pos")
    idx = torch.empty(m_total, dtype=_i32, device=pos.device)
    B = ptr.numel() - 1
    for t, name in ((gap_out, "gap_out"), (nested_gap, "nested_gap")):
        if t is not None:
            _chk(t, torch.float32, name)
    nbytes = _lib.load().gn_fps_workspace_bytes(B, int(max_points))
    ws = torch.empty(nbytes, dtype=torch.uint8, device=pos.device) if nbytes else None
    _lib.call("gn_fps_nested_ws", _p(pos), _p(ptr), _p(out_ptr), _p(start_idx), B, int(max_points), _p(idx), _p(gap_out), _p(nested_gap),
              _p(ws), nbytes, _stream())
    return idx


def ball_query(pos, ptr, centre_idx, centre_ptr, r, K=64):
    M = centre_idx.numel()
    nbr = torch.empty((M, K), dtype=_i32, device=pos.device)
    cnt = torch.empty(M, dtype=_i32, device=pos.device)
    r2 = float(np.float32(float(r) * float(r)))
    _lib.call("gn_ball_query", _p(pos), _p(ptr), _p(centre_idx), _p(centre_ptr), ptr.numel() - 1, M, r2, K, _p(nbr), _p(cnt), _stream())
    return nbr, cnt


def sa_gather(x, pos, centre_idx, nbr, self_loops=True, self_src=None):
    M, K = nbr.shape
    C = 0 if x is None else x.shape[1]
    S = K + (1 if self_loops else 0)
    out = new_rows(M * S, C + 3, pos.device)
    slot_src = torch.empty(M * S, dtype=_i32, device=pos.device)
    ldx = 0 if x is None else rows_view(x)[1]
    _lib.call("gn_sa_gather_scoped", _p(x), ldx, C, _p(pos), _p(centre_idx), _p(nbr), M, K, 1 if self_loops else 0,
              _p(_chk(self_src, _i32, "self_src") if self_src is not None else None), _p(out), out.stride(0), _p(slot_src), _stream())
    return out, slot_src, S


def segment_max(h, slot_src, M, S):
    C = h.shape[1]
    out = new_rows(M, C, h.device)
    _lib.call("gn_segment_max", _p(h), rows_view(h)[1], _p(slot_src), M, S, C, _p(out), out.stride(0), _stream())
    return out


class SaFusedPack:

    def __init__(self, w1p, w2p, w3p, tab, cin, dims):
        self.w1p, self.w2p, self.w3p, self.tab, self.cin, self.dims = w1p, w2p, w3p, tab, int(cin), tuple(int(v) for v in dims)
        self.cout = self.dims[2]
        self.macs_per_edge = (self.cin + 3) * self.dims[0] + self.dims[0] * self.dims[1] + self.dims[1] * self.dims[2]

    def to(self, device):
        return SaFusedPack(self.w1p.to(device), self.w2p.to(device), self.w3p.to(device), self.tab.to(device), self.cin, self.dims)


def sa_fused_supported(cin, dims):
    return len(dims) == 3 and bool(_lib.load().gn_sa_fused_supported(int(cin), int(dims[0]), int(dims[1]), int(dims[2])))


def pack_sa_fused(layers):
    ar = torch.arange
    packs, tabs, dims = [], [], []
    for w, b, sc, sh in layers:
        w = w.detach().float().cpu()
        n, k = w.shape
        assert n % 32 == 0
        kb_n = (((k + 7) // 8 * 8) + 31) // 32
        wz = torch.zeros((n, kb_n * 32), dtype=torch.float32)
        wz[:, :k] = w
        nb, kb, qq, h, r, i = torch.meshgrid(ar(n // 32), ar(kb_n), ar(4), ar(2), ar(32), ar(4), indexing="ij")
        packs.append(wz[32 * nb + r, 32 * kb + 8 * qq + 4 * h + i].contiguous())
        nbt, ht, q = torch.meshgrid(ar(n // 32), ar(2), ar(16), indexing="ij")
        u = 32 * nbt + 8 * (q >> 2) + (q & 3) + 4 * ht
        one = lambda v, fill: (torch.full((n,), fill) if v is None else v.detach().float().cpu())
        tabs.append(torch.stack((one(b, 0.0)[u], one(sc, 1.0)[u], one(sh, 0.0)[u]), dim=2).reshape(-1))
        dims.append(n)
    cin = layers[0][0].shape[1] - 3
    return SaFusedPack(packs[0], packs[1], packs[2], torch.cat(tabs).contiguous(), cin, dims)


def sa_fused(x, pos, centre_idx, nbr, cnt, pack, self_loops=True, self_src=None, group=0, out=None):
    M, K = nbr.shape
    if out is None:
        out = new_rows(M, pack.cout, pos.device)
    elif out.dtype != torch.float32 or tuple(out.shape) != (M, pack.cout):
        raise ValueError(f"sa_fused: out must be float32 [{M}][{pack.cout}]")
    ldx = 0 if x is None else rows_view(x)[1]
    _lib.call("gn_sa_fused_group", _p(x), ldx, pack.cin, _p(_chk(pos, torch.float32, "pos")), _p(centre_idx), _p(nbr), _p(cnt), M, K, 1 if self_loops else 0,
              _p(_chk(self_src, _i32, "self_src") if self_src is not None else None), _p(pack.w1p), _p(pack.w2p), _p(pack.w3p), _p(pack.tab), pack.dims[0], pack.dims[1], pack.dims[2], _p(out), rows_view(out)[1], _stream(),
              int(group))
    return out


def sa_fused_auto_group(cin, dims, M):
    g = _lib.load().gn_sa_fused_auto_group(int(cin), int(dims[0]), int(dims[1]), int(dims[2]), int(M))
    if g <= 0:
        raise ValueError(f"sa_fused_auto_group: {_lib.load().gn_last_error().decode(errors='replace')}")
    return g


def global_max_pool(h, ptr, B):
    C = h.shape[1]
    out = new_rows(B, C, h.device)
    _lib.call("gn_global_max_pool", _p(h), rows_view(h)[1], _p(ptr), B, C, _p(out), out.stride(0), _stream())
    return out


KNN_MAXK = 8


def knn_interpolate(xs, ps, ptr_s, pq, ptr_q, k, out=None):
    Nq, C = pq.shape[0], xs.shape[1]
    if out is None:
        out = new_rows(Nq, C, xs.device)
    _lib.call("gn_knn_interpolate" if int(k) <= KNN_MAXK else "gn_knn_interpolate_any", _p(xs), rows_view(xs)[1], _p(ps), _p(ptr_s), _p(pq), _p(ptr_q),
              ptr_s.numel() - 1, Nq, C, int(k), _p(out), rows_view(out)[1], _stream())
    return out


def linear(x, w, bias=None, bn_scale=None, bn_shift=None, relu=False, out=None, K=None):
    M = x.shape[0]
    K = x.shape[1] if K is None else K
    N = w.shape[0]
    if out is None:
        out = new_rows(M, N, x.device)
    _lib.call("gn_linear", _p(x), rows_view(x)[1], _p(w), rows_view(w)[1], _p(bias), _p(bn_scale), _p(bn_shift), 1 if relu else 0,
              M, N, K, _p(out), rows_view(out)[1], _stream())
    return out


def nocs_head(logits, bins):
    N = logits.shape[0]
    dev = logits.device
    idx = torch.empty((N, 3), dtype=torch.int64, device=dev)
    conf = torch.empty((N, 3), dtype=torch.float32, device=dev)
    nocs = torch.empty((N, 3), dtype=torch.float32, device=dev)
    _lib.call("gn_nocs_head", _p(logits), rows_view(logits)[1], N, bins, _p(idx), _p(conf), _p(nocs), _stream())
    return idx, conf, nocs


def _f3(v):
    return (ctypes.c_float * 3)(*[float(a) for a in v])


def _i3(v):
    return (ctypes.c_int * 3)(*[int(a) for a in v])


def grid_features(feat, nocs, sim_pos, conf, batch, lower, upper, grid_shape, include_point=True, include_conf=True):
    N, Cf = feat.shape
    C = Cf + (6 if include_point else 0) + (3 if include_conf else 0)
    out = new_rows(N, C, feat.device)
    flat = torch.empty(N, dtype=_i32, device=feat.device)
    _lib.call("gn_grid_features", _p(feat), rows_view(feat)[1], Cf, _p(_chk(nocs, torch.float32, "nocs")),
              _p(_chk(sim_pos, torch.float32, "sim_pos")), _p(_chk(conf, torch.float32, "conf")), _p(_chk(batch, torch.int64, "batch")),
              N, _f3(lower), _f3(upper), _i3(grid_shape), 1 if include_point else 0, 1 if include_conf else 0, _p(out),
              out.stride(0), _p(flat), _stream())
    return out, flat


def zeroed_volume(B, grid_shape, C, device):
    vol = torch.zeros((B,) + tuple(grid_shape) + (C,), dtype=torch.float32, device=device)
    cnt = torch.zeros(B * int(np.prod(grid_shape)), dtype=_i32, device=device)
    return vol, cnt


REDUCE_CODES = {"max": 0, "mean": 1, "sum": 2, "add": 2, "min": 3, "mul": 4}


def grid_scatter(src, flat_idx, B, grid_shape, reduce, with_stats=False, prezeroed=None, c_real=None):
    N, C = src.shape
    if reduce not in REDUCE_CODES:
        raise ValueError(f"grid_scatter: reduce={reduce!r} is not one of {sorted(REDUCE_CODES)}")
    if with_stats and reduce == "mul":
        raise ValueError("grid_scatter: the occupied-cell statistics assume empty cells are 0, which 'mul' leaves at 1")
    cps = int(np.prod(grid_shape))
    cells = B * cps
    if prezeroed is not None:
        vol, cnt = prezeroed
        assert vol.shape == (B,) + tuple(grid_shape) + (C,) and cnt.numel() == cells
    else:
        vol = torch.empty((B,) + tuple(grid_shape) + (C,), dtype=torch.float32, device=src.device)
        cnt = torch.empty(cells, dtype=_i32, device=src.device)
    code = REDUCE_CODES[reduce]
    nbytes = _lib.load().gn_grid_scatter_workspace_bytes(N, C, code)
    ws = torch.empty(nbytes, dtype=torch.uint8, device=src.device) if nbytes else None
    _lib.call("gn_grid_scatter_ex", _p(src), rows_view(src)[1], _p(flat_idx), N, C, C if c_real is None else int(c_real), cells, code, _p(vol), _p(cnt),
              _p(ws), nbytes, 0 if prezeroed is None else 1, _stream())
    if not with_stats:
        return vol
    s, q = _stats_buffers(B, C, src.device, True)
    _lib.call("gn_grid_stats", _p(vol), _p(flat_idx), N, C, cps, B, _p(cnt), _p(s), _p(q), _stream())
    return vol, (s, q, cps)


def channel_stats(x):
    B, C = x.shape[0], x.shape[-1]
    V = x.numel() // (B * C)
    s, q = _stats_buffers(B, C, x.device, True)
    narrow = (C <= 256 and 256 % C == 0) or C % 256 == 0
    _lib.call("gn_channel_stats" if narrow else "gn_channel_stats_any", _p(x), B, V, C, _p(s), _p(q), _stream())
    return s, q, V


def groupnorm_affine(st0, st1, groups, eps, gamma, beta, with_act_scale=False, real=None):
    s0, q0, V0 = st0
    B, C0 = s0.shape
    if st1 is not None:
        s1, q1, V1 = st1
        C1 = s1.shape[1]
        rep = V0 // V1
    else:
        s1 = q1 = None
        C1, V1, rep = 0, 0, 1
    a = torch.empty((B, C0 + C1), dtype=torch.float32, device=s0.device)
    d = torch.empty_like(a)
    inv = torch.empty(B, dtype=torch.float32, device=s0.device) if with_act_scale else None
    r0, r1 = (C0, C1) if real is None else (int(real[0]), int(real[1]) if len(real) > 1 else 0)
    if (r0, r1) == (C0, C1) and C0 + C1 <= GNA_MAXC:
        _lib.call("gn_groupnorm_affine", _p(s0), _p(q0), C0, V0, _p(s1), _p(q1), C1, V1, rep, B, groups, float(eps), _p(gamma), _p(beta),
                  _p(a), _p(d), _p(inv), _stream())
    else:
        _lib.call("gn_groupnorm_affine_map", _p(s0), _p(q0), r0, C0, V0, _p(s1), _p(q1), r1, C1, V1, rep, B, groups, float(eps), _p(gamma),
                  _p(beta), _p(a), _p(d), _p(inv), _stream())
    return (a, d, inv) if with_act_scale else (a, d)


GNA_MAXC = 1024


def pack_conv_weight(w):
    cout, cin = w.shape[:2]
    assert cin % 16 == 0
    return w.detach().float().permute(2, 3, 4, 1, 0).reshape(27, cin // 16, 16, cout).permute(0, 1, 3, 2).contiguous()


from .arith import CONV_FP32, CONV_MODE_NAMES, SPLIT_BF16X2, SPLIT_BF16X3, SPLIT_F16X2


class SplitPack:

    def __init__(self, tensor, mode, out_scale):
        self.tensor, self.mode, self.out_scale = tensor, int(mode), out_scale

    def to(self, device):
        return SplitPack(self.tensor.to(device), self.mode, self.out_scale.to(device))


def pack_conv_weight_split(w, mode):
    if mode not in (SPLIT_BF16X2, SPLIT_BF16X3, SPLIT_F16X2):
        raise ValueError(f"unknown split mode {mode}")
    cout, cin = w.shape[:2]
    w = w.detach().float()
    planes, dt = (2, torch.float16) if mode == SPLIT_F16X2 else (int(mode), torch.bfloat16)
    scale = torch.ones(cout, dtype=torch.float32)
    if mode == SPLIT_F16X2:
        m = w.reshape(cout, -1).abs().amax(dim=1).cpu()
        ok = torch.isfinite(m) & (m > 0)
        scale = torch.where(ok, torch.exp2(-torch.floor(torch.log2(torch.where(ok, m, torch.ones_like(m))))), scale).float()
    base = (w * scale.to(w.device).view(cout, 1, 1, 1, 1)).permute(2, 3, 4, 1, 0).reshape(27, cin // 16, 2, 8, cout // 32, 32)
    base = base.permute(1, 0, 4, 2, 5, 3)
    out, r = [], base
    for _ in range(planes):
        p = r.to(dt)
        out.append(p)
        r = r - p.float()
    pk = torch.stack(out, dim=3).contiguous()
    pk = pk.reshape(cin // 16 * 27, -1)
    pk = torch.cat([pk, torch.zeros_like(pk[:1]).repeat(8, 1)], dim=0)
    return SplitPack(pk.contiguous().view(torch.int16), mode, (1.0 / scale).contiguous().to(w.device))


def wino_supported(cin, cout, dims):
    D, H, W = [int(v) for v in dims]
    if not (cin % 16 == 0 and cout % 32 == 0 and H % 8 == 0 and W % 8 == 0 and D * H * W <= (1 << 27) and D * H * W * cin * 4 < (1 << 32)):
        return False
    return (cin <= 256 and D % 4 == 0) if cout % 128 == 0 else (cin <= 128 and D % 8 == 0)


def pack_conv_weight_split_wino(w):
    cout, cin = w.shape[:2]
    w = w.detach().double().cpu()
    G = torch.tensor([[1.0, 0.0, 0.0], [0.5, 0.5, 0.5], [0.5, -0.5, 0.5], [0.0, 0.0, 1.0]], dtype=torch.float64)
    u = torch.einsum("jk,nczyk->nczyj", G, w)
    m = u.reshape(cout, -1).abs().amax(dim=1)
    scale = _pow2_floor_inv(m)
    base = (u * scale.view(cout, 1, 1, 1, 1)).float().permute(4, 2, 3, 1, 0).reshape(36, cin // 16, 2, 8, cout // 32, 32)
    base = base.permute(1, 0, 4, 2, 5, 3)
    p1 = base.to(torch.float16)
    p2 = (base - p1.float()).to(torch.float16)
    pk = torch.stack((p1, p2), dim=3).contiguous().reshape(cin // 16 * 36, -1)
    pk = torch.cat([pk, torch.zeros_like(pk[:6])], dim=0)
    return SplitPack(pk.contiguous().view(torch.int16), SPLIT_F16X2, (1.0 / scale).float().contiguous())


def conv3d_gcr_split_wino(src, a, d, pack, cout, relu=True, with_stats=False, act_inv=None, tile_active=None, kconst=None, kreach=1, partial=None):
    return _conv3d_wino("conv3d_gcr_split_wino", src, a, d, pack.tensor, pack.out_scale, act_inv, None, cout, relu, with_stats, tile_active, kconst, kreach,
                        partial)


def _conv3d_wino(who, src, a, d, pack, out_scale, act_inv, kbias, cout, relu, with_stats, tile_active, kconst, kreach, partial):
    B, D, H, W, C0 = src.shape
    if partial is not None and tile_active is not None:
        raise ValueError(f"{who}: the occupancy-aware launch cannot take a polyphase partial")
    out, s, q, ows, ows_bytes = _conv_outputs(src, cout, with_stats, tile_active)
    if partial is not None:
        _lib.call("gn_conv3d_gcr_split_wino_partial", _p(src), C0, _p(a), _p(d), _p(pack), _p(out_scale), _p(act_inv), _p(kbias), B, D, H, W, cout,
                  1 if relu else 0, _p(out), _p(s), _p(q), _p(_chk(partial, torch.float32, "partial")), _stream())
    else:
        _lib.call("gn_conv3d_gcr_split_wino", _p(src), C0, _p(a), _p(d), _p(pack), _p(out_scale), _p(act_inv), _p(kbias), B, D, H, W, cout,
                  1 if relu else 0, _p(out), _p(s), _p(q), _p(tile_active), _p(kconst), int(kreach), _p(ows), ows_bytes, _stream())
    return (out, (s, q, D * H * W)) if with_stats else out


def grid_tile_flags(flat_idx, B, grid_shape, reach=1):
    g0, g1, g2 = [int(v) for v in grid_shape]
    tiles = -(-g0 // 4) * -(-g1 // 8) * -(-g2 // 8)
    flags = torch.empty((B, tiles), dtype=torch.uint8, device=flat_idx.device)
    _lib.call("gn_grid_tile_flags", _p(_chk(flat_idx, _i32, "flat_idx")), flat_idx.numel(), B, g0, g1, g2, int(reach), _p(flags), _stream())
    return flags


def polyphase_weights(w, c0):
    w = w.detach().double().cpu()
    cout = w.shape[0]
    w0, w1 = w[:, :c0].float(), w[:, c0:]
    M = torch.zeros(2, 3, 3, dtype=torch.float64)
    M[0, 0, 0] = M[0, 1, 1] = M[0, 1, 2] = 1.0
    M[1, 1, 0] = M[1, 1, 1] = M[1, 2, 2] = 1.0
    blocks = [torch.einsum("az,by,cx,nkzyx->nkabc", M[pz], M[py], M[px], w1) for pz in (0, 1) for py in (0, 1) for px in (0, 1)]
    wm = torch.cat(blocks, dim=0).float()
    nz = (wm.reshape(8 * cout // 32, 32, -1, 27) != 0).any(dim=2).any(dim=1)
    mask = torch.zeros(27, dtype=torch.int64)
    for blk in range(nz.shape[0]):
        mask |= nz[blk].to(torch.int64) << blk
    return w0.contiguous(), wm.contiguous(), mask.to(torch.int32)


def pack_upconv_weight(wm, cout, mode):
    if mode not in (SPLIT_BF16X2, SPLIT_F16X2):
        raise ValueError("gn_upconv_partial runs the two-plane modes only")
    wm = wm.detach().float().cpu()
    c1 = wm.shape[1]
    assert wm.shape[0] == 8 * cout and c1 % 16 == 0 and cout % 32 == 0
    taps = torch.empty((8, 8, cout, c1), dtype=torch.float32)
    for c in range(8):
        pz, py, px = c >> 2, (c >> 1) & 1, c & 1
        for t in range(8):
            iz, iy, ix = t >> 2, (t >> 1) & 1, t & 1
            taps[c, t] = wm[c * cout:(c + 1) * cout, :, pz + iz, py + iy, px + ix]
    scale = torch.ones(8, cout)
    if mode == SPLIT_F16X2:
        m = taps.abs().amax(dim=(1, 3))
        ok = torch.isfinite(m) & (m > 0)
        scale = torch.where(ok, torch.exp2(-torch.floor(torch.log2(torch.where(ok, m, torch.ones_like(m))))), scale)
    dt = torch.float16 if mode == SPLIT_F16X2 else torch.bfloat16
    t_ = (taps * scale[:, None, :, None]).reshape(8, 8, cout // 32, 32, c1 // 16, 2, 8)
    t_ = t_.permute(4, 1, 0, 2, 5, 3, 6)
    p1 = t_.to(dt)
    p2 = (t_ - p1.float()).to(dt)
    pk = torch.stack((p1, p2), dim=4).contiguous()
    return SplitPack(pk.view(torch.int16).reshape(-1), mode, (1.0 / scale).reshape(-1).contiguous())


def _device_pack_args(who, w, c_lo, c_n):
    if not isinstance(w, torch.Tensor) or w.dim() != 5 or tuple(w.shape[2:]) != (3, 3, 3):
        raise ValueError(f"{who}: expected a Conv3d weight (Cout, Cin, 3, 3, 3)")
    if w.dtype != torch.float32:
        raise ValueError(f"{who}: expected torch.float32, got {w.dtype}")
    if not w.is_contiguous():
        raise ValueError(f"{who}: the weight must be contiguous")
    cout, cin = int(w.shape[0]), int(w.shape[1])
    c_lo = int(c_lo)
    c_n = cin - c_lo if c_n is None else int(c_n)
    if c_lo < 0 or c_n <= 0 or c_lo + c_n > cin:
        raise ValueError(f"{who}: input channels [{c_lo}, {c_lo + c_n}) outside the weight's {cin}")
    if c_n % 16 != 0 or cout % 32 != 0:
        raise ValueError(f"{who}: channels must be multiples of 16 (in) / 32 (out), got {c_n} / {cout}")
    if not w.is_cuda:
        raise ValueError(f"{who}: the weight must be on the GPU (the host builder takes a CPU tensor)")
    return w.detach(), cout, cin, c_lo, c_n


def pack_conv_weight_split_device(w, mode, c_lo=0, c_n=None):
    if mode not in (SPLIT_BF16X2, SPLIT_BF16X3, SPLIT_F16X2):
        raise ValueError(f"unknown split mode {mode}")
    w, cout, cin, c_lo, c_n = _device_pack_args("pack_conv_weight_split_device", w, c_lo, c_n)
    planes = 2 if mode == SPLIT_F16X2 else int(mode)
    pk = torch.empty((c_n // 16 * 27 + 8, cout // 32 * planes * 512), dtype=torch.int16, device=w.device)
    scale = torch.empty((cout,), dtype=torch.float32, device=w.device)
    _lib.call("gn_weight_pack_split", _p(w), cout, cin, c_lo, c_n, int(mode), _p(pk), pk.numel() * 2, _p(scale), _stream())
    return SplitPack(pk, mode, scale)

# ... 1736 lines not shown
```

### include/garmentnets_hip.h

```cpp
#ifndef GARMENTNETS_HIP_H
#define GARMENTNETS_HIP_H

#include <stddef.h>
#include <stdint.h>

#ifdef __cplusplus
extern "C" {
#endif

#define GN_OK 0
#define GN_EINVAL (-1)
#define GN_ELAUNCH (-2)
#define GN_ECAP (-3)

const char *gn_last_error(void);
int gn_version(void);
const char *gn_last_kernel(void);
int gn_device_info(int *num_cu, int *lds_bytes_per_cu);


int gn_segment_ptr(const int64_t *batch, int64_t n, int B, int32_t *ptr, void *stream);

int gn_fps(const float *pos, const int32_t *ptr, const int32_t *out_ptr, const int32_t *start_idx, int B,
           int max_points_per_example, int32_t *out_idx, void *stream);

int gn_fps_nested(const float *pos, const int32_t *ptr, const int32_t *out_ptr, const int32_t *start_idx, int B,
                  int max_points_per_example, int32_t *out_idx, float *gap_out, const float *nested_gap, void *stream);
size_t gn_fps_workspace_bytes(int B, int max_points_per_example);
int gn_fps_nested_ws(const float *pos, const int32_t *ptr, const int32_t *out_ptr, const int32_t *start_idx, int B,
                     int max_points_per_example, int32_t *out_idx, float *gap_out, const float *nested_gap, void *ws, size_t ws_bytes,
                     void *stream);

int gn_ball_query(const float *pos, const int32_t *ptr, const int32_t *centre_idx, const int32_t *centre_ptr, int B,
                  int M, float r2, int K, int32_t *nbr, int32_t *cnt, void *stream);

int gn_sa_gather(const float *x, int ldx, int C, const float *pos, const int32_t *centre_idx, const int32_t *nbr,
                 int M, int K, int self_loops, float *out, int ldo, int32_t *slot_src, void *stream);
int gn_sa_gather_scoped(const float *x, int ldx, int C, const float *pos, const int32_t *centre_idx, const int32_t *nbr,
                        int M, int K, int self_loops, const int32_t *self_src, float *out, int ldo, int32_t *slot_src, void *stream);

int gn_segment_max(const float *in, int ldi, const int32_t *slot_src, int M, int S, int C, float *out, int ldo,
                   void *stream);

int gn_sa_fused_supported(int C, int N1, int N2, int N3);
int gn_sa_fused(const float *x, int ldx, int C, const float *pos, const int32_t *centre_idx, const int32_t *nbr, const int32_t *cnt,
                int M, int K, int self_loops, const float *w1p, const float *w2p, const float *w3p, const float *tab, int N1, int N2,
                int N3, float *out, int ldo, void *stream);
int gn_sa_fused_scoped(const float *x, int ldx, int C, const float *pos, const int32_t *centre_idx, const int32_t *nbr, const int32_t *cnt,
                       int M, int K, int self_loops, const int32_t *self_src, const float *w1p, const float *w2p, const float *w3p,
                       const float *tab, int N1, int N2, int N3, float *out, int ldo, void *stream);
int gn_sa_fused_group(const float *x, int ldx, int C, const float *pos, const int32_t *centre_idx, const int32_t *nbr, const int32_t *cnt,
                      int M, int K, int self_loops, const int32_t *self_src, const float *w1p, const float *w2p, const float *w3p,
                      const float *tab, int N1, int N2, int N3, float *out, int ldo, void *stream, int group);
int gn_sa_fused_auto_group(int C, int N1, int N2, int N3, int M);

int gn_global_max_pool(const float *in, int ldi, const int32_t *ptr, int B, int C, float *out, int ldo, void *stream);

int gn_knn_interpolate(const float *xs, int ldx, const float *ps, const int32_t *ptr_s, const float *pq,
                       const int32_t *ptr_q, int B, int Nq, int C, int k, float *out, int ldo, void *stream);
int gn_knn_interpolate_any(const float *xs, int ldx, const float *ps, const int32_t *ptr_s, const float *pq,
                           const int32_t *ptr_q, int B, int Nq, int C, int k, float *out, int ldo, void *stream);

int gn_linear(const float *X, int ldx, const float *W, int ldw, const float *bias, const float *bn_scale,
              const float *bn_shift, int relu, int64_t M, int N, int K, float *Y, int ldy, void *stream);

int gn_nocs_head(const float *logits, int ldl, int64_t N, int bins, int64_t *bin_idx , float *confidence ,
                 float *pred_nocs , void *stream);


int gn_grid_features(const float *feat, int ldf, int Cf, const float *nocs, const float *sim_pos, const float *conf,
                     const int64_t *batch, int64_t N, const float lower[3], const float upper[3], const int grid[3],
                     int include_point, int include_conf, float *out, int ldo, int32_t *flat_idx, void *stream);

size_t gn_grid_scatter_workspace_bytes(int64_t N, int C, int reduce);
int gn_grid_scatter(const float *src, int lds, const int32_t *flat_idx, int64_t N, int C, int64_t cells, int reduce,
                    float *vol, int32_t *count_ws, void *ws, size_t ws_bytes, int vol_is_zeroed, void *stream);
int gn_grid_scatter_ex(const float *src, int lds, const int32_t *flat_idx, int64_t N, int C, int c_real, int64_t cells, int reduce,
                       float *vol, int32_t *count_ws, void *ws, size_t ws_bytes, int vol_is_zeroed, void *stream);

int gn_grid_tile_flags(const int32_t *flat_idx, int64_t N, int B, int G0, int G1, int G2, int reach, unsigned char *flags, void *stream);

int gn_grid_stats(const float *vol, const int32_t *flat_idx, int64_t N, int C, int64_t cells_per_sample, int B,
                  int32_t *count_ws, double *sum, double *sumsq, void *stream);


int gn_channel_stats(const float *x, int B, int64_t V, int C, double *sum, double *sumsq, void *stream);

int gn_channel_stats_any(const float *x, int B, int64_t V, int C, double *sum, double *sumsq, void *stream);

int gn_groupnorm_affine(const double *sum0, const double *sq0, int C0, int64_t V0, const double *sum1, const double *sq1,
                        int C1, int64_t V1, int rep1, int B, int groups, float eps, const float *gamma,
                        const float *beta, float *a, float *d, float *act_inv_scale, void *stream);

int gn_groupnorm_affine_map(const double *sum0, const double *sq0, int C0, int S0, int64_t V0, const double *sum1, const double *sq1,
                            int C1, int S1, int64_t V1, int rep1, int B, int groups, float eps, const float *gamma,
                            const float *beta, float *a, float *d, float *act_inv_scale, void *stream);

int gn_conv3d_gcr(const float *src0, int C0, const float *src1, int C1, const float *a, const float *d,
                  const float *wp, int B, int D, int H, int W, int Cout, int relu, float *out, double *out_sum,
                  double *out_sumsq, void *stream);

#define GN_SPLIT_BF16X2 2
#define GN_SPLIT_BF16X3 3
#define GN_SPLIT_F16X2 4
size_t gn_conv3d_occupancy_workspace_bytes(int B, int D, int H, int W);
int gn_conv3d_gcr_split(const float *src0, int C0, const float *src1, int C1, const float *a, const float *d,
                        const void *wp_planes, int mode, const float *out_scale, const float *act_inv_scale, int B, int D, int H, int W,
                        int Cout, int relu, float *out, double *out_sum, double *out_sumsq, const unsigned char *tile_active,
                        const float *kconst, int kreach, const float *partial, void *occ_ws, size_t occ_ws_bytes, void *stream);

size_t gn_conv_affine_pack_bytes(int B, int Cin, int Cout);
int gn_conv_affine_pack(const float *w, int Cin, int Cout, const float *a, const float *d, const double *sum, const double *sumsq, int64_t V,
                        const float *coff, int B, void *pack, size_t pack_bytes, float *stage_a, float *stage_d, float *out_scale,
                        float *kbias, void *ws, size_t ws_bytes, void *stream);
int gn_conv3d_gcr_split_persample(const float *src, int Cin, const float *stage_a, const float *stage_d, const void *pack,
                                  const float *out_scale, const float *kbias, int B, int D, int H, int W, int Cout, int relu, float *out,
                                  double *out_sum, double *out_sumsq, const unsigned char *tile_active, const float *kconst, int kreach,
                                  const float *partial, void *occ_ws, size_t occ_ws_bytes, void *stream);

size_t gn_conv_affine_pack_wino_bytes(int B, int Cin, int Cout);
int gn_conv_affine_pack_wino(const float *w, int Cin, int Cout, const float *a, const float *d, const double *sum, const double *sumsq, int64_t V,
                             const float *coff, int B, void *pack, size_t pack_bytes, float *stage_a, float *stage_d, float *out_scale,
                             float *kbias, void *ws, size_t ws_bytes, void *stream);
int gn_conv3d_gcr_split_wino(const float *src, int Cin, const float *a, const float *d, const void *pack, const float *out_scale,
                             const float *act_inv_scale, const float *kbias, int B, int D, int H, int W, int Cout, int relu, float *out,
                             double *out_sum, double *out_sumsq, const unsigned char *tile_active, const float *kconst, int kreach,
                             void *occ_ws, size_t occ_ws_bytes, void *stream);
int gn_conv3d_gcr_split_wino_partial(const float *src, int Cin, const float *a, const float *d, const void *pack, const float *out_scale,
                                     const float *act_inv_scale, const float *kbias, int B, int D, int H, int W, int Cout, int relu, float *out,
                                     double *out_sum, double *out_sumsq, const float *partial, void *stream);

int gn_upconv_partial(const float *src1, int C1, const float *a, const float *d, const void *wp, int mode, const float *out_scale,
                      const float *act_inv_scale, int B, int Dc, int Hc, int Wc, int Cout, float *partial, void *stream);

size_t gn_weight_pack_split_bytes(int c_n, int Cout, int mode);
size_t gn_weight_pack_split_wino_bytes(int c_n, int Cout);
size_t gn_weight_pack_upconv_bytes(int C1, int Cout);
int gn_weight_pack_split(const float *w, int Cout, int Cin, int c_lo, int c_n, int mode, void *pack, size_t pack_bytes, float *out_scale,
                         void *stream);
int gn_weight_pack_split_wino(const float *w, int Cout, int Cin, int c_lo, int c_n, void *pack, size_t pack_bytes, float *out_scale,
                              void *stream);
int gn_weight_pack_upconv(const float *w, int Cout, int Cin, int c0, int mode, void *pack, size_t pack_bytes, float *out_scale, void *stream);

int gn_affine_act(const float *x, int B, int64_t V, int C, const float *a, const float *d, const float *bias, int act, float *out, void *stream);

int gn_maxpool3d_2(const float *in, int B, int D, int H, int W, int C, float *out, double *out_sum, double *out_sumsq,
                   void *stream);

int gn_trilinear_sample(const float *vol, int D, int H, int W, int C, const float *query, int Q, int64_t m0, int64_t M,
                        float *out, int ldo, void *stream);
int gn_trilinear_sample_batch(const float *vol, int B, int64_t vol_bstride, int D, int H, int W, int C, const float *query, int64_t M, float *out, int ldo,
                              void *stream);

int gn_implicit_decode(const float *vol, int D, int H, int W, int C0, const float *xin, int ldxin, const float *query, int Q, int64_t m0, int64_t M,
                       const float *w1p, const float *b1, const float *s1, const float *t1, int N1, const float *w2p,
                       const float *b2, const float *s2, const float *t2, int N2, const float *w3, const float *b3,
                       const float *s3, const float *t3, int OUT, float *out, int ldo, const float *run_if, void *stream);


int gn_ggm3d(const float *vol, int n0, int n1, int n2, double sigma, float *tmp, float *out, void *stream);

int gn_minmax(const float *x, int64_t n, float *out2, void *stream);
int gn_ggm3d_batch(const float *vol, int batch, int n0, int n1, int n2, double sigma, float *tmp, float *out, void *stream);
int gn_minmax_batch(const float *x, int batch, int64_t n, float *out2, void *stream);
size_t gn_ggm3d_range_workspace_bytes(int batch, int n0, int n1, int n2);
int gn_ggm3d_batch_ex(const float *vol, int batch, int n0, int n1, int n2, double sigma, float *tmp, float *out, int accum_bits, float *range2,
                      void *range_ws, size_t range_ws_bytes, void *stream);

size_t gn_mc33_workspace_bytes(int n0, int n1, int n2);
int gn_mc33(const float *vol, int n0, int n1, int n2, double level, void *ws, size_t ws_bytes, float *verts,
            int32_t *faces, float *normals, float *values, int64_t cap_v, int64_t cap_f, int64_t *counts_dev,
            void *stream);
size_t gn_mc33_batch_workspace_bytes(int batch, int n0, int n1, int n2);
int gn_mc33_batch(const float *vol, int batch, int n0, int n1, int n2, double level, void *ws, size_t ws_bytes, float *verts,
                  int32_t *faces, float *normals, float *values, int64_t cap_v, int64_t cap_f, int64_t *counts_dev, void *stream);
int gn_mc33_batch_profiled(const float *vol, int batch, int n0, int n1, int n2, double level, void *ws, size_t ws_bytes, float *verts,
                           int32_t *faces, float *normals, float *values, int64_t cap_v, int64_t cap_f, int64_t *counts_dev, void *stream,
                           float *stage_ms);

int gn_gather_nn(const float *vol, int n0, int n1, int n2, const float *verts_vox, int64_t nv, double spacing,
                 float *out, void *stream);
int gn_gather_nn_batch(const float *vol, int batch, int n0, int n1, int n2, const float *verts_vox, int64_t nv, double spacing,
                       float *out, void *stream);

int gn_scale_verts(const float *verts_vox, int64_t nv, double spacing, float *verts_out, void *stream);

size_t gn_mesh_compact_workspace_bytes(int64_t V, int64_t F);
int gn_mesh_compact(const void *verts, int vert_bytes, const int32_t *faces, const unsigned char *on_surface, int64_t V, int64_t F,
                    void *ws, size_t ws_bytes, void *out_verts, int32_t *out_faces, int64_t *counts, void *stream);

size_t gn_mesh_largest_component_workspace_bytes(int64_t V);
int gn_mesh_largest_component(const int32_t *faces, int64_t F, int64_t V, void *ws, size_t ws_bytes, unsigned char *mask, int32_t *label,
                              int64_t *info, void *stream);

int gn_implicit_decode_split(const float *xin, int ldxin, int64_t M, const void *wpack, const float *tab, const float *xscale,
                             int C0, int N1, int N2, int OUT, float *out, int ldo, void *stream);
int gn_implicit_decode_split_batch(const float *xin, int ldxin, int64_t M, int B, const void *wpack, const float *tab, const float *xscale,
                                   int C0, int N1, int N2, int OUT, float *out, int ldo, void *stream);
int gn_implicit_decode_batch(const float *xin, int ldxin, int64_t M, int B, int C0, const float *w1p, const float *b1, const float *s1, const float *t1,
                             int N1, const float *w2p, const float *b2, const float *s2, const float *t2, int N2, const float *w3, const float *b3,
                             const float *s3, const float *t3, int OUT, float *out, int ldo, const float *run_if, int run_if_stride, void *stream);

int gn_implicit_decode_lattice_split(const float *vol, int D, int H, int W, int C0, int Q, int64_t m0, int64_t M, const void *wpack,
                                     const float *tab, const float *xscale, int N1, int N2, int OUT, float *out, int ldo, void *stream);

int gn_decoder_input_scale(const double *sumsq, int64_t V, int B, int C, float smax, float *out4, void *stream);


int gn_nearest_neighbor(const float *query, int64_t nq, const float *ref, int64_t nr, int32_t *idx, float *d2, void *stream);

int gn_nearest_neighbor_f64_batch(const double *query, const double *ref, const int64_t *pairs, int P, int64_t max_nq, int32_t *idx, double *d2,
                                  void *stream);

int gn_point_mesh_sqdist_batch(const double *query, const double *verts, const int32_t *faces, const int64_t *pairs, int P, int64_t max_nq,
                               int32_t *face_idx, double *d2, int64_t *bad, void *stream);


int gn_winding_number_batch(const double *query, const double *verts, const int32_t *faces, const int64_t *pairs, int P, int64_t max_nq,
                            double *out, int64_t *bad, void *stream);

int gn_winding_field_batch(const double *verts, const int32_t *faces, const int64_t *mesh_csr, int B, int D, int H, int W, float *out,
                           int64_t *bad, void *stream);

int gn_distance_field_batch(const double *verts, const int32_t *faces, const int64_t *mesh_csr, int B, int D, int H, int W,
                            int32_t *face_idx, double *d2, int64_t *bad, void *stream);

#define GN_QT_FACE_CHUNK 512
#define GN_QT_WINDING 0
#define GN_QT_DISTANCE 1
#define GN_QT_SIGNED_DISTANCE 2
#define GN_QT_OCCUPANCY 3

int gn_query_targets_face_chunk(void);
size_t gn_query_targets_workspace_bytes(int B, int64_t M, int64_t max_nf, int kind);
int gn_query_targets_batch(const float *query, const float *verts, const int32_t *faces, const int64_t *mesh_csr, int B, int64_t M, int64_t max_nf, int kind,
                           int use_clip, float tsdf_clip, int absolute, void *ws, size_t ws_bytes, float *target, double *w, double *d2, int32_t *face_idx,
                           int64_t *bad, void *stream);

#define GN_LOSS_MAX_SETS 8
#define GN_LOSS_L2 0
#define GN_LOSS_SMOOTH_L1 1
#define GN_LOSS_BCE_LOGITS 2
#define GN_LOSS_ROW_NORM 3

typedef struct {
    const float *logits;
    const float *gt;
    int64_t n;
    int ldl;
    int pad;
} GnNocsBinSet;

typedef struct {
    const float *pred;
    const float *target;
    int64_t count;
    int kind;
    int mirror;
} GnLossSegment;

size_t gn_nocs_bin_metrics_workspace_bytes(const GnNocsBinSet *sets_host, int nsets);
int gn_nocs_bin_metrics(const GnNocsBinSet *sets_host, int nsets, int bins, int mirror_axis, void *ws, size_t ws_bytes, double *out, void *stream);

size_t gn_value_losses_workspace_bytes(const GnLossSegment *segs_host, int nsegs);
int gn_value_losses(const GnLossSegment *segs_host, int nsegs, void *ws, size_t ws_bytes, double *out, void *stream);

typedef struct {
    const float *logits;
    const float *gt;
    float *grad;
    int64_t n;
    int ldl;
    int ldg;
    int ncols;
    int pad;
} GnNocsBinGradSet;

typedef struct {
    const float *pred;
    const float *target;
    float *grad;
    int64_t count;
    double coef;
    int kind;
    int mirror;
} GnLossGradSegment;

int gn_nocs_bin_loss_bwd(const GnNocsBinGradSet *sets_host, int nsets, int bins, int mirror_axis, const double *sums, const double *weights_host,
                         const float *upstream, void *stream);

int gn_value_losses_bwd(const GnLossGradSegment *segs_host, int nsegs, const double *sums, const float *upstream, void *stream);

#define GN_ADAM_CHUNK 4096
#define GN_ADAM_MAX_HYPER 16
typedef struct {
    float *p;
    const float *g;
    float *exp_avg;
    float *exp_avg_sq;
    int64_t numel;
    int64_t blk0;
    int hyper;
    int pad;
} GnAdamEntry;

typedef struct {
    double lr, beta1, beta2, eps, weight_decay;
    double bias_correction1;
    double bias_correction2_sqrt;
} GnAdamHyper;

int gn_adam_step(const GnAdamEntry *table, int n, int64_t nblocks, const GnAdamHyper *hyper_host, int nhyper, void *stream);

typedef struct {
    const void *src;
    int64_t dst_off;
    int64_t numel;
    int64_t blk0;
} GnPackEntry;

int gn_grad_pack(const GnPackEntry *table, int n_entries, int64_t n_blocks, float *flat, int64_t flat_numel, int world, void *stream);


size_t gn_grid_scatter_bwd_workspace_bytes(int64_t N, int C, int64_t cells, int reduce);
int gn_grid_scatter_bwd(const float *grad_vol, const float *vol, const float *src, int lds, const int32_t *flat_idx, int64_t N, int C, int c_real,
                        int64_t cells, int reduce, void *ws, size_t ws_bytes, float *grad_src, int ldg, void *stream);

int gn_segment_max_bwd(const float *grad_out, int ldg, const float *out, int ldo, const float *in, int ldi, const int32_t *slot_src, int M, int S,
                       int C, float *grad_in, int ldgi, void *stream);

int gn_global_max_pool_bwd(const float *grad_out, int ldg, const float *out, int ldo, const float *in, int ldi, const int32_t *ptr, int B, int C,
                           float *grad_in, int ldgi, void *stream);

size_t gn_sa_gather_bwd_workspace_bytes(int64_t rows, int64_t n_points);
int gn_sa_gather_bwd(const float *grad_edge, int lde, const int32_t *slot_src, int64_t rows, int C, int64_t n_points, void *ws, size_t ws_bytes,
                     float *grad_x, int ldgx, void *stream);

int gn_knn_neighbours(const float *ps, const int32_t *ptr_s, const float *pq, const int32_t *ptr_q, int B, int Nq, int k, int32_t *nbr, float *d2,
                      void *stream);
size_t gn_knn_interpolate_bwd_workspace_bytes(int64_t Nq, int k, int64_t Ns);
int gn_knn_interpolate_bwd(const int32_t *nbr, const float *d2, int Nq, int k, const float *grad_y, int ldg, int Ns, int C, void *ws, size_t ws_bytes,
                           float *grad_xs, int ldgx, void *stream);

size_t gn_trilinear_sample_bwd_workspace_bytes(int B, int64_t M, int D, int H, int W);
int gn_trilinear_sample_bwd(const float *grad_rows, int ldg, const float *vol, int B, int D, int H, int W, int C, const float *query, int64_t M,
                            void *ws, size_t ws_bytes, float *grad_vol, float *grad_query, void *stream);


size_t gn_conv3d_bwd_weight_workspace_bytes(int B, int D, int H, int W, int Cin, int Cout);
int gn_conv3d_bwd_weight(const float *src0, int C0, const float *src1, int C1, const float *a, const float *d, const float *y, const float *dy,
                         int B, int D, int H, int W, int Cout, void *ws, size_t ws_bytes, float *dw, void *stream);

int gn_relu_mask(const float *y, const float *dy, int64_t n, float *g, void *stream);


size_t gn_relu_mask_max_workspace_bytes(int B);
// ... 169 lines not shown
```

Before: 157.4.

## Overlap chunked FPS with ball query and fused SA on a side stream

Result: no change. 158.5, median of 6 (+0.7%).

```diff
diff --git a/garmentnets_amd/_lib.py b/garmentnets_amd/_lib.py
--- a/garmentnets_amd/_lib.py
+++ b/garmentnets_amd/_lib.py
@@ -17,7 +17,11 @@
     "gn_fps_nested": [_vp, _vp, _vp, _vp, _i32, _i32, _vp, _vp, _vp, _vp],
     "gn_fps_workspace_bytes": [_i32, _i32],
     "gn_fps_nested_ws": [_vp, _vp, _vp, _vp, _i32, _i32, _vp, _vp, _vp, _vp, _sz, _vp],
+    "gn_fps_resume_state_bytes": [_i32, _i32],
+    "gn_fps_resume": [_vp, _vp, _vp, _vp, _i32, _i32, _vp, _vp, _vp, _vp, _sz, _vp],
     "gn_ball_query": [_vp, _vp, _vp, _vp, _i32, _i32, _f32, _i32, _vp, _vp, _vp],
+    "gn_ball_query_rows": [_vp, _vp, _vp, _vp, _i32, _i32, _f32, _i32, _vp, _vp, _vp, _i32, _vp],
+    "gn_sa_fused_rows": [_vp, _i32, _i32, _vp, _vp, _vp, _vp, _i32, _i32, _i32, _vp, _vp, _vp, _vp, _vp, _i32, _i32, _i32, _vp, _i32, _vp, _i32, _vp, _i32],
     "gn_sa_gather": [_vp, _i32, _i32, _vp, _vp, _vp, _i32, _i32, _i32, _vp, _i32, _vp, _vp],
     "gn_segment_max": [_vp, _i32, _vp, _i32, _i32, _i32, _vp, _i32, _vp],
     "gn_sa_fused_supported": [_i32, _i32, _i32, _i32],
@@ -161,7 +165,7 @@
                                          _i32, _vp, _vp, _vp, _vp],
 }
 _RESTYPES = {"gn_weight_pack_split_bytes": _sz, "gn_weight_pack_split_wino_bytes": _sz, "gn_weight_pack_upconv_bytes": _sz,
-             "gn_conv_affine_pack_bytes": _sz, "gn_conv_affine_pack_wino_bytes": _sz, "gn_conv3d_occupancy_workspace_bytes": _sz, "gn_mc33_workspace_bytes": _sz, "gn_ggm3d_range_workspace_bytes": _sz, "gn_mc33_batch_workspace_bytes": _sz, "gn_grid_scatter_workspace_bytes": _sz, "gn_fps_workspace_bytes": _sz, "gn_mesh_compact_workspace_bytes": _sz, "gn_mesh_largest_component_workspace_bytes": _sz,
+             "gn_conv_affine_pack_bytes": _sz, "gn_conv_affine_pack_wino_bytes": _sz, "gn_conv3d_occupancy_workspace_bytes": _sz, "gn_mc33_workspace_bytes": _sz, "gn_ggm3d_range_workspace_bytes": _sz, "gn_mc33_batch_workspace_bytes": _sz, "gn_grid_scatter_workspace_bytes": _sz, "gn_fps_workspace_bytes": _sz, "gn_fps_resume_state_bytes": _sz,"gn_mesh_compact_workspace_bytes": _sz, "gn_mesh_largest_component_workspace_bytes": _sz,
              "gn_nocs_bin_metrics_workspace_bytes": _sz, "gn_value_losses_workspace_bytes": _sz,
              "gn_grid_scatter_bwd_workspace_bytes": _sz, "gn_sa_gather_bwd_workspace_bytes": _sz, "gn_knn_interpolate_bwd_workspace_bytes": _sz,
              "gn_trilinear_sample_bwd_workspace_bytes": _sz, "gn_conv3d_bwd_weight_workspace_bytes": _sz, "gn_conv3d_bwd_weight_split_workspace_bytes": _sz, "gn_relu_mask_max_workspace_bytes": _sz, "gn_groupnorm_bwd_stats_workspace_bytes": _sz,
diff --git a/garmentnets_amd/components/pointnet2.py b/garmentnets_amd/components/pointnet2.py
--- a/garmentnets_amd/components/pointnet2.py
+++ b/garmentnets_amd/components/pointnet2.py
@@ -9,6 +9,8 @@
 from .mlp import fold_batchnorm, generation, param_cache
 
 FUSED_SA = os.environ.get("GARMENTNETS_FUSED_SA", "1") != "0"
+FPS_OVERLAP = os.environ.get("GARMENTNETS_FPS_OVERLAP", "1") != "0"
+FPS_CHUNKS = 4
 
 class _DeviceTableCache:
 
@@ -42,6 +44,44 @@
     return _SELF_SRC_CACHE.get((tuple(sizes), tuple(centre_sizes), str(device)), build)
 
 
+def fps_chunk_ranges(sizes, centre_sizes, C):
+    if len(sizes) != len(centre_sizes) or int(C) < 1:
+        raise ValueError("fps_chunk_ranges: one centre count per example and at least one chunk")
+    out = []
+    for n, m in zip(sizes, centre_sizes):
+        steps = max(int(m) - 1, 0) if n > 0 else 0
+        cb = min(int(C), steps)
+        out.append([(1 + c * steps // cb, 1 + (c + 1) * steps // cb) for c in range(cb)])
+    return out
+
+
+def fps_chunk_tables(sizes, centre_sizes, C):
+    ranges = fps_chunk_ranges(sizes, centre_sizes, C)
+    starts = np.concatenate([[0], np.cumsum(centre_sizes)]).astype(np.int64)
+    tables = []
+    for c in range(int(C)):
+        steps, rows = np.zeros((len(sizes), 2), dtype=np.int32), []
+        for b, (n, m) in enumerate(zip(sizes, centre_sizes)):
+            m = int(m) if n > 0 else 0
+            k0, k1 = ranges[b][c] if c < len(ranges[b]) else (m, m)
+            if c == 0:
+                k0 = 0
+            steps[b] = (k0, k1)
+            rows.append(starts[b] + np.arange(k0, k1))
+        tables.append((steps, np.concatenate(rows or [np.zeros(0)]).astype(np.int32)))
+    return tables
+
+
+_CHUNK_TABLE_CACHE = _DeviceTableCache()
+_SIDE = threading.local()
+
+
+def _chunk_tables(sizes, centre_sizes, C, device):
+    def build():
+        return [(torch.from_numpy(s).to(device), torch.from_numpy(r).to(device)) for s, r in fps_chunk_tables(sizes, centre_sizes, C)]
+    return _CHUNK_TABLE_CACHE.get((tuple(sizes), tuple(centre_sizes), int(C), str(device)), build)
+
+
 class Segments:
 
     def __init__(self, sizes, device, batch=None):
@@ -94,6 +134,7 @@
         self.max_num_neighbors = max_num_neighbors
         self.conv = PointConv(nn)
         self.random_start = random_start
+        self.fps_chunks = None
 
     def forward(self, x, pos, batch):
         seg = Segments.of(batch)
@@ -108,23 +149,66 @@
             src = getattr(pos, "_fps_cascade", None)
             if src is not None and src[1] == seg.sizes and src[2] == pos._version and src[0].device == pos.device:
                 nested = src[0]
-        idx = ops.fps(pos, seg.ptr, cseg.ptr, max(seg.sizes) if seg.sizes else 0, cseg.total, start, gap_out=gap, nested_gap=nested)
-        nbr, cnt = ops.ball_query(pos, seg.ptr, idx, cseg.ptr, self.r, self.max_num_neighbors)
         pack = self._fused_pack() if FUSED_SA else None
+        if pack is not None and not ((x is None and pack.cin == 0) or (x is not None and x.shape[1] == pack.cin)):
+            pack = None
         self_src = None
         if self.conv.add_self_loops and self.conv.self_loop_scope == "example" and seg.num > 1:
             self_src = _example_self_src(seg.sizes, out_sizes, pos.device)
-        if pack is not None and ((x is None and pack.cin == 0) or (x is not None and x.shape[1] == pack.cin)):
-            out = ops.sa_fused(x, pos, idx, nbr, cnt, pack, self_loops=self.conv.add_self_loops, self_src=self_src)
+        chunks = self._overlap_chunks(x, pos, seg, out_sizes, nested, pack)
+        if chunks > 1:
+            idx, nbr, cnt, out = self._forward_overlapped(x, pos, seg, cseg, start, gap, pack, self_src, chunks)
         else:
-            edges, slot_src, S = ops.sa_gather(x, pos, idx, nbr, self_loops=self.conv.add_self_loops, self_src=self_src)
-            h = self.conv.local_nn(edges)
-            out = ops.segment_max(h, slot_src, cseg.total, S)
+            idx = ops.fps(pos, seg.ptr, cseg.ptr, max(seg.sizes) if seg.sizes else 0, cseg.total, start, gap_out=gap, nested_gap=nested)
+            nbr, cnt = ops.ball_query(pos, seg.ptr, idx, cseg.ptr, self.r, self.max_num_neighbors)
+            if pack is not None:
+                out = ops.sa_fused(x, pos, idx, nbr, cnt, pack, self_loops=self.conv.add_self_loops, self_src=self_src)
+            else:
+                edges, slot_src, S = ops.sa_gather(x, pos, idx, nbr, self_loops=self.conv.add_self_loops, self_src=self_src)
+                h = self.conv.local_nn(edges)
+                out = ops.segment_max(h, slot_src, cseg.total, S)
         _DEBUG.__dict__.setdefault("graphs", weakref.WeakKeyDictionary())[self] = (idx, nbr)
         pos_out = pos[idx.long()]
         if gap is not None:
             pos_out._fps_cascade = (gap, out_sizes, pos_out._version)
         return out, pos_out, cseg
+
+    def _overlap_chunks(self, x, pos, seg, out_sizes, nested, pack):
+        C = int(self.fps_chunks or FPS_CHUNKS)
+        if not FPS_OVERLAP or C < 2 or pack is None or nested is not None or seg.num == 0 or min(out_sizes) < C:
+            return 1
+        if torch.is_grad_enabled() and (pos.requires_grad or (x is not None and x.requires_grad) or any(p.requires_grad for p in self.parameters())):
+            return 1
+        if torch.cuda.is_current_stream_capturing():
+            return 1
+        if not ops.fps_resume_state_bytes(seg.num, max(seg.sizes)):
+            return 1
+        return C
+
+    def _forward_overlapped(self, x, pos, seg, cseg, start, gap, pack, self_src, C):
+        dev, M, K = pos.device, cseg.total, self.max_num_neighbors
+        tables = _chunk_tables(seg.sizes, cseg.sizes, C, dev)
+        max_points = max(seg.sizes)
+        idx = torch.empty(M, dtype=torch.int32, device=dev)
+        nbr = torch.empty((M, K), dtype=torch.int32, device=dev)
+        cnt = torch.empty(M, dtype=torch.int32, device=dev)
+        out = ops.new_rows(M, pack.cout, dev)
+        state = torch.empty(ops.fps_resume_state_bytes(seg.num, max_points), dtype=torch.uint8, device=dev)
+        main = torch.cuda.current_stream(dev)
+        streams = _SIDE.__dict__.setdefault("streams", {})
+        side = streams.get(dev)
+        if side is None:
+            side = streams[dev] = torch.cuda.Stream(device=dev)
+        for steps, rows in tables:
+            ops.fps_resume(pos, seg.ptr, cseg.ptr, max_points, idx, steps, state, start_idx=start, gap_out=gap)
+            done = torch.cuda.Event()
+            done.record(main)
+            side.wait_event(done)
+            with torch.cuda.stream(side):
+                ops.ball_query_rows(pos, seg.ptr, idx, cseg.ptr, self.r, nbr, cnt, rows)
+                ops.sa_fused_rows(x, pos, idx, nbr, cnt, pack, out, rows, self_loops=self.conv.add_self_loops, self_src=self_src)
+        main.wait_stream(side)
+        return idx, nbr, cnt, out
 
     @property
     def last_graph(self):
diff --git a/garmentnets_amd/csrc/points.hip b/garmentnets_amd/csrc/points.hip
--- a/garmentnets_amd/csrc/points.hip
+++ b/garmentnets_amd/csrc/points.hip
@@ -53,6 +53,9 @@
 
 #define FPS_THREADS 1024
 #define FPS_WAVES (FPS_THREADS / 64)
+#ifndef FPS_MID_THREADS
+#define FPS_MID_THREADS 512
+#endif
 
 __device__ __forceinline__ float fps_min(float a, float b) {
     float o;
@@ -81,11 +84,13 @@
     return __builtin_amdgcn_readfirstlane(fi);
 }
 
-template <int PPT, bool LDS_POS, int THREADS>
+#define FPS_STATE_FLOATS(PPT, THREADS) ((PPT) * (THREADS) + 4)
+template <int PPT, bool LDS_POS, int THREADS, bool RESUME = false>
 __global__ __launch_bounds__(THREADS) void fps_kernel(const float *__restrict__ pos, const int32_t *__restrict__ ptr,
                                                       const int32_t *__restrict__ out_ptr, const int32_t *__restrict__ start_idx,
                                                       int32_t *__restrict__ out_idx, float *__restrict__ gap_out,
-                                                      const float *__restrict__ nested_gap) {
+                                                      const float *__restrict__ nested_gap, float *__restrict__ state,
+                                                      const int32_t *__restrict__ steps) {
     constexpr int WAVES = THREADS / 64;
     static_assert(PPT == 1 || PPT % 2 == 0, "points are updated in pairs");
     extern __shared__ __attribute__((aligned(16))) float smem[];
@@ -93,6 +98,12 @@
     const int s = ptr[b], n = ptr[b + 1] - s;
     const int o0 = out_ptr[b], m = out_ptr[b + 1] - o0;
     if (n <= 0 || m <= 0) return;
+    int k0 = 0, k1 = m;
+    if (RESUME) {
+        k0 = steps[2 * b] > 0 ? steps[2 * b] : 0;
+        k1 = steps[2 * b + 1] < m ? steps[2 * b + 1] : m;
+        if (k0 >= k1) return;
+    }
     const int tid = threadIdx.x, lane = tid & 63, wave = tid >> 6;
     if (nested_gap && nested_gap[b] > 0.f && m <= n) {
         for (int k = tid; k < m; k += THREADS) out_idx[o0 + k] = s + k;
@@ -122,8 +133,16 @@
     if (LDS_POS) __syncthreads();
     int last = start_idx ? start_idx[b] : 0;
     if (last < 0 || last >= n) last = 0;
-    if (tid == 0) out_idx[o0] = s + last;
-    for (int k = 1; k < m; ++k) {
+    float *const st = RESUME ? state + (size_t)b * FPS_STATE_FLOATS(PPT, THREADS) : nullptr;
+    if (RESUME && k0 > 0) {
+#pragma unroll
+        for (int j = 0; j < PPT; ++j) dd[j] = st[j * THREADS + tid];
+        last = __float_as_int(st[PPT * THREADS]);
+        gmin = st[PPT * THREADS + 1];
+    } else if (tid == 0) {
+        out_idx[o0] = s + last;
+    }
+    for (int k = RESUME ? (k0 > 1 ? k0 : 1) : 1; k < (RESUME ? k1 : m); ++k) {
         float qx, qy, qz;
         if (LDS_POS) { qx = lx[last]; qy = ly[last]; qz = lz[last]; }
         else { qx = gp[3 * last]; qy = gp[3 * last + 1]; qz = gp[3 * last + 2]; }
@@ -152,6 +171,12 @@
         last = fps_pick<WAVES, true>(bv, bi, k, pv, pi, lane, wave, gv);
         gmin = fps_min(gmin, gv);
         if (tid == 0) out_idx[o0 + k] = s + last;
+    }
+    if (RESUME && k1 < m) {
+#pragma unroll
+        for (int j = 0; j < PPT; ++j) st[j * THREADS + tid] = dd[j];
+        if (tid == 0) { st[PPT * THREADS] = __int_as_float(last); st[PPT * THREADS + 1] = gmin; }
+        return;
     }
     if (gap_out && tid == 0) gap_out[b] = gmin;
 }
@@ -217,11 +242,31 @@
     return (size_t)B * (size_t)max_points_per_example * sizeof(float4);
 }
 
+static void fps_resident_shape(int n, int *threads, int *ppt) {
+    static const int inst[] = {2, 4, 6, 8, 12, 16, 24};
+    *threads = n <= 24 * 256 ? 256 : (n <= 24 * FPS_MID_THREADS ? FPS_MID_THREADS : FPS_THREADS);
+    const int need = (int)gn_cdiv(n, *threads);
+    *ppt = 24;
+    for (int i = 6; i >= 0; --i)
+        if (need <= inst[i]) *ppt = inst[i];
+    if (*threads == FPS_THREADS) *ppt = 16;
+}
+
+extern "C" size_t gn_fps_resume_state_bytes(int B, int max_points_per_example) {
+    if (B <= 0 || max_points_per_example <= 0 || max_points_per_example > 16 * FPS_THREADS) return 0;
+    int threads, ppt;
+    fps_resident_shape(max_points_per_example, &threads, &ppt);
+    return (size_t)B * FPS_STATE_FLOATS(ppt, threads) * sizeof(float);
+}
+
 static int fps_checked_launch(const float *pos, const int32_t *ptr, const int32_t *out_ptr, const int32_t *start_idx, int B, int n, int32_t *out_idx,
-                              float *gap_out, const float *nested_gap, bool takes_ws, void *ws, size_t ws_bytes, void *stream) {
+                              float *gap_out, const float *nested_gap, bool takes_ws, void *ws, size_t ws_bytes, void *stream,
+                              float *state = nullptr, const int32_t *steps = nullptr) {
     GN_REQUIRE(B >= 0 && n >= 0, "gn_fps: bad sizes");
     GN_REQUIRE(nested_gap == nullptr || start_idx == nullptr, "gn_fps_nested: a nested sample starts at the example's first point (start_idx must be NULL)");
     if (B == 0 || n == 0) return GN_OK;
+    GN_REQUIRE(steps == nullptr || n <= 16 * FPS_THREADS, "gn_fps_resume: only the register-resident sampler resumes (at most %d points per example, got %d)",
+               16 * FPS_THREADS, n);
     if (n > FPS_LDS_MAX) {
         GN_REQUIRE(takes_ws, "gn_fps: more than %d points per example needs a workspace: gn_fps_nested_ws (got %d)", FPS_LDS_MAX, n);
         const size_t need = gn_fps_workspace_bytes(B, n);
@@ -242,16 +287,20 @@
         return GN_OK;
     }
     const bool lds_pos = n <= 8192;
-#ifndef FPS_MID_THREADS
-#define FPS_MID_THREADS 512
-#endif
-    const int threads = n <= 24 * 256 ? 256 : (n <= 24 * FPS_MID_THREADS ? FPS_MID_THREADS : FPS_THREADS);
+    int threads, ppt;
+    fps_resident_shape(n, &threads, &ppt);
     size_t sh = sizeof(float) * 4 * (threads / 64) + (lds_pos ? sizeof(float) * 3 * (size_t)n : 0);
-    const int ppt = (int)gn_cdiv(n, threads);
 #define FPS_LAUNCH(P, L, T)                                                                                     \
     do {                                                                                                        \
+        if (steps) {                                                                                            \
+            GN_HIP(hipFuncSetAttribute((const void *)fps_kernel<P, L, T, true>, hipFuncAttributeMaxDynamicSharedMemorySize, (int)sh), "gn_fps_resume"); \
+            hipLaunchKernelGGL((fps_kernel<P, L, T, true>), dim3(B), dim3(T), sh, gn_stream(stream), pos, ptr, out_ptr, start_idx, out_idx, gap_out, \
+                               (const float *)nullptr, state, steps);                                           \
+            break;                                                                                              \
+        }                                                                                                       \
         GN_HIP(hipFuncSetAttribute((const void *)fps_kernel<P, L, T>, hipFuncAttributeMaxDynamicSharedMemorySize, (int)sh), "gn_fps"); \
-        hipLaunchKernelGGL((fps_kernel<P, L, T>), dim3(B), dim3(T), sh, gn_stream(stream), pos, ptr, out_ptr, start_idx, out_idx, gap_out, nested_gap); \
+        hipLaunchKernelGGL((fps_kernel<P, L, T>), dim3(B), dim3(T), sh, gn_stream(stream), pos, ptr, out_ptr, start_idx, out_idx, gap_out, nested_gap, \
+                           (float *)nullptr, (const int32_t *)nullptr);                                         \
     } while (0)
 #define FPS_BY_PPT(L, T)                               \
     do {                                               \
@@ -289,13 +338,31 @@
     return fps_checked_launch(pos, ptr, out_ptr, start_idx, B, max_points_per_example, out_idx, gap_out, nested_gap, true, ws, ws_bytes, stream);
 }
 
+extern "C" int gn_fps_resume(const float *pos, const int32_t *ptr, const int32_t *out_ptr, const int32_t *start_idx, int B,
+                             int max_points_per_example, int32_t *out_idx, float *gap_out, const int32_t *steps, void *state, size_t state_bytes,
+                             void *stream) {
+    GN_REQUIRE(B >= 0 && max_points_per_example >= 0, "gn_fps_resume: bad sizes");
+    if (B == 0 || max_points_per_example == 0) return GN_OK;
+    const size_t need = gn_fps_resume_state_bytes(B, max_points_per_example);
+    GN_REQUIRE(need > 0, "gn_fps_resume: only the register-resident sampler resumes (at most %d points per example, got %d)", 16 * FPS_THREADS,
+               max_points_per_example);
+    GN_REQUIRE(steps != nullptr, "gn_fps_resume: steps is NULL");
+    GN_REQUIRE(state != nullptr && state_bytes >= need, "gn_fps_resume: the state needs %zu bytes (gn_fps_resume_state_bytes), got %zu", need,
+               state ? state_bytes : (size_t)0);
+    return fps_checked_launch(pos, ptr, out_ptr, start_idx, B, max_points_per_example, out_idx, gap_out, nullptr, false, nullptr, 0, stream,
+                              reinterpret_cast<float *>(state), steps);
+}
+
 __global__ __launch_bounds__(256) void ball_query_kernel(const float *__restrict__ pos, const int32_t *__restrict__ ptr,
                                                          const int32_t *__restrict__ centre_idx,
                                                          const int32_t *__restrict__ centre_ptr, int B, int M, float r2, int K,
-                                                         int32_t *__restrict__ nbr, int32_t *__restrict__ cnt) {
+                                                         int32_t *__restrict__ nbr, int32_t *__restrict__ cnt,
+                                                         const int32_t *__restrict__ rows, int R) {
     const int lane = threadIdx.x & 63;
-    const int c = blockIdx.x * (blockDim.x >> 6) + (threadIdx.x >> 6);
-    if (c >= M) return;
+    const int w = blockIdx.x * (blockDim.x >> 6) + (threadIdx.x >> 6);
+    if (w >= R) return;
+    const int c = rows ? rows[w] : w;
+    if ((unsigned)c >= (unsigned)M) return;
     int lo = 0, hi = B;
     while (hi - lo > 1) {
         int mid = (lo + hi) >> 1;
@@ -329,8 +396,19 @@
     GN_REQUIRE(B >= 0 && M >= 0 && K > 0, "gn_ball_query: bad sizes");
     if (M == 0) return GN_OK;
     hipLaunchKernelGGL(ball_query_kernel, dim3((unsigned)gn_cdiv(M, 4)), dim3(256), 0, gn_stream(stream), pos, ptr, centre_idx,
-                       centre_ptr, B, M, r2, K, nbr, cnt);
+                       centre_ptr, B, M, r2, K, nbr, cnt, (const int32_t *)nullptr, M);
     GN_LAUNCH_CHECK("gn_ball_query");
+    return GN_OK;
+}
+
+extern "C" int gn_ball_query_rows(const float *pos, const int32_t *ptr, const int32_t *centre_idx, const int32_t *centre_ptr, int B, int M,
+                                  float r2, int K, int32_t *nbr, int32_t *cnt, const int32_t *rows, int R, void *stream) {
+    GN_REQUIRE(B >= 0 && M >= 0 && K > 0 && R >= 0 && R <= M, "gn_ball_query_rows: bad sizes");
+    if (R == 0) return GN_OK;
+    GN_REQUIRE(rows != nullptr, "gn_ball_query_rows: rows is NULL");
+    hipLaunchKernelGGL(ball_query_kernel, dim3((unsigned)gn_cdiv(R, 4)), dim3(256), 0, gn_stream(stream), pos, ptr, centre_idx,
+                       centre_ptr, B, M, r2, K, nbr, cnt, rows, R);
+    GN_LAUNCH_CHECK("gn_ball_query_rows");
     return GN_OK;
 }
 
diff --git a/garmentnets_amd/csrc/sa_fused.hip b/garmentnets_amd/csrc/sa_fused.hip
--- a/garmentnets_amd/csrc/sa_fused.hip
+++ b/garmentnets_amd/csrc/sa_fused.hip
@@ -11,6 +11,7 @@
     const float4 *w1, *w2, *w3;
     const float *tab;
     float *out; int ldo;
+    const int32_t *rows; int R;
 };
 
 __device__ __forceinline__ f32x16 sa_mfma(float a, float b, const f32x16 &c) { return __builtin_amdgcn_mfma_f32_32x32x2f32(a, b, c, 0, 0, 0); }
@@ -54,7 +55,7 @@
     }
 }
 
-template <int CIN, int N1, int N2, int N3, int G>
+template <int CIN, int N1, int N2, int N3, int G, bool ROWS = false>
 __global__ __launch_bounds__(256, 2) void sa_fused_kernel(SaArgs p) {
     constexpr int K1 = CIN + 3, K1P = (K1 + 7) & ~7, KB1 = (K1P + 31) / 32;
     constexpr int LASTQ1 = (K1P - 32 * (KB1 - 1)) / 8;
@@ -66,6 +67,7 @@
     __shared__ int tile_ctr;
     const int tid = threadIdx.x, lane = tid & 63, h = lane >> 5, r = lane & 31;
     const int c0 = blockIdx.x * G;
+    const int lim = ROWS ? p.R : p.M;
     for (int i = tid; i < G * N3; i += 256) out_lds[i] = gn_sord_enc(-INFINITY);
     for (int i = tid; i < TABN; i += 256) tab[i] = p.tab[i];
     if (tid == 0) tile_ctr = 0;
@@ -80,16 +82,17 @@
         int j, ci, cl;
         if (t < 2 * G) {
             cl = t >> 1;
-            const int c = c0 + cl, half = t & 1;
-            if (c >= p.M) continue;
+            const int w = c0 + cl, half = t & 1;
+            if (w >= lim) continue;
+            const int c = ROWS ? p.rows[w] : w;
             if (p.cnt[c] <= 32 * half) continue;
             const int slot = 32 * half + r;
             j = slot < p.K ? p.nbr[(size_t)c * p.K + slot] : -1;
             if (p.self_loops && j == (p.self_src ? p.self_src[c] : c)) j = -1;
             ci = p.centre_idx[c];
         } else {
-            const int c = c0 + r;
-            const bool ok = r < G && c < p.M;
+            const bool ok = r < G && c0 + r < lim;
+            const int c = ROWS ? (ok ? p.rows[c0 + r] : 0) : c0 + r;
             cl = r;
             j = ok ? (p.self_src ? p.self_src[c] : c) : -1;
             ci = ok ? p.centre_idx[c] : 0;
@@ -169,8 +172,9 @@
     }
     __syncthreads();
     for (int i = tid; i < G * N3; i += 256) {
-        const int cl = i / N3, u = i % N3, c = c0 + cl;
-        if (c < p.M) {
+        const int cl = i / N3, u = i % N3;
+        if (c0 + cl < lim) {
+            const int c = ROWS ? p.rows[c0 + cl] : c0 + cl;
             const float v = gn_sord_dec(out_lds[i]);
             p.out[(size_t)c * p.ldo + u] = v == -INFINITY ? 0.f : v;
         }
@@ -208,13 +212,19 @@
 }
 template <int CIN, int N1, int N2, int N3>
 static int sa_launch(const SaArgs &p, hipStream_t st, int group) {
-    switch (group ? group : sa_auto_group<CIN, N1, N2, N3>(p.M)) {
-        case 32: hipLaunchKernelGGL((sa_fused_kernel<CIN, N1, N2, N3, 32>), dim3((unsigned)gn_cdiv(p.M, 32)), dim3(256), 0, st, p); break;
-        case 16: hipLaunchKernelGGL((sa_fused_kernel<CIN, N1, N2, N3, 16>), dim3((unsigned)gn_cdiv(p.M, 16)), dim3(256), 0, st, p); break;
-        case 8: hipLaunchKernelGGL((sa_fused_kernel<CIN, N1, N2, N3, 8>), dim3((unsigned)gn_cdiv(p.M, 8)), dim3(256), 0, st, p); break;
-        case 4: hipLaunchKernelGGL((sa_fused_kernel<CIN, N1, N2, N3, 4>), dim3((unsigned)gn_cdiv(p.M, 4)), dim3(256), 0, st, p); break;
-        default: hipLaunchKernelGGL((sa_fused_kernel<CIN, N1, N2, N3, 2>), dim3((unsigned)gn_cdiv(p.M, 2)), dim3(256), 0, st, p); break;
-    }
+#define SA_GO(g, grid)                                                                                             \
+    do {                                                                                                           \
+        if (p.rows) hipLaunchKernelGGL((sa_fused_kernel<CIN, N1, N2, N3, g, true>), grid, dim3(256), 0, st, p);    \
+        else hipLaunchKernelGGL((sa_fused_kernel<CIN, N1, N2, N3, g>), grid, dim3(256), 0, st, p);                 \
+    } while (0)
+    switch (group ? group : sa_auto_group<CIN, N1, N2, N3>(p.R)) {
+        case 32: SA_GO(32, dim3((unsigned)gn_cdiv(p.R, 32))); break;
+        case 16: SA_GO(16, dim3((unsigned)gn_cdiv(p.R, 16))); break;
+        case 8: SA_GO(8, dim3((unsigned)gn_cdiv(p.R, 8))); break;
+        case 4: SA_GO(4, dim3((unsigned)gn_cdiv(p.R, 4))); break;
+        default: SA_GO(2, dim3((unsigned)gn_cdiv(p.R, 2))); break;
+    }
+#undef SA_GO
     return 0;
 }
 
@@ -239,20 +249,22 @@
     return GN_EINVAL;
 }
 
-extern "C" int gn_sa_fused_group(const float *x, int ldx, int C, const float *pos, const int32_t *centre_idx, const int32_t *nbr,
-                                 const int32_t *cnt, int M, int K, int self_loops, const int32_t *self_src, const float *w1p,
-                                 const float *w2p, const float *w3p, const float *tab, int N1, int N2, int N3, float *out, int ldo,
-                                 void *stream, int group) {
+static int sa_checked_launch(const float *x, int ldx, int C, const float *pos, const int32_t *centre_idx, const int32_t *nbr,
+                             const int32_t *cnt, int M, int K, int self_loops, const int32_t *self_src, const float *w1p,
+                             const float *w2p, const float *w3p, const float *tab, int N1, int N2, int N3, float *out, int ldo,
+                             void *stream, int group, const int32_t *rows, int R) {
     GN_REQUIRE(M >= 0 && K > 0 && K <= 64 && ldo >= N3, "gn_sa_fused: bad sizes (the ball-query table holds at most 64 neighbours)");
     GN_REQUIRE(group == 0 || group == 2 || group == 4 || group == 8 || group == 16 || group == 32, "gn_sa_fused: group %d is not one of 0 (the cost rule), 2, 4, 8, 16, 32", group);
     GN_REQUIRE(gn_sa_fused_supported(C, N1, N2, N3), "gn_sa_fused: edge MLP [%d+3,%d,%d,%d] is not instantiated (see SA_SHAPES in csrc/sa_fused.hip); use gn_sa_gather + gn_linear + gn_segment_max", C, N1, N2, N3);
     GN_REQUIRE(C == 0 || (x && ldx >= C && (C < 8 || (ldx % 4 == 0 && (uintptr_t)x % 16 == 0))), "gn_sa_fused: feature rows need a 16-byte aligned base and leading dimension");
-    if (M == 0) return GN_OK;
+    GN_REQUIRE(R >= 0 && R <= M, "gn_sa_fused_rows: %d rows of %d centres", R, M);
+    if (R == 0) return GN_OK;
     GN_REQUIRE(pos && centre_idx && nbr && cnt && w1p && w2p && w3p && tab && out, "gn_sa_fused: null pointer");
     SaArgs p;
     p.x = x; p.ldx = ldx; p.pos = pos; p.centre_idx = centre_idx; p.nbr = nbr; p.cnt = cnt; p.M = M; p.K = K; p.self_loops = self_loops;
     p.self_src = self_src;
     p.w1 = (const float4 *)w1p; p.w2 = (const float4 *)w2p; p.w3 = (const float4 *)w3p; p.tab = tab; p.out = out; p.ldo = ldo;
+    p.rows = rows; p.R = R;
     hipStream_t st = gn_stream(stream);
 #define SA_DISPATCH(c, n1, n2, n3) if (C == c && N1 == n1 && N2 == n2 && N3 == n3) sa_launch<c, n1, n2, n3>(p, st, group);
     SA_SHAPES(SA_DISPATCH)
@@ -261,6 +273,23 @@
     return GN_OK;
 }
 
+extern "C" int gn_sa_fused_group(const float *x, int ldx, int C, const float *pos, const int32_t *centre_idx, const int32_t *nbr,
+                                 const int32_t *cnt, int M, int K, int self_loops, const int32_t *self_src, const float *w1p,
+                                 const float *w2p, const float *w3p, const float *tab, int N1, int N2, int N3, float *out, int ldo,
+                                 void *stream, int group) {
+    return sa_checked_launch(x, ldx, C, pos, centre_idx, nbr, cnt, M, K, self_loops, self_src, w1p, w2p, w3p, tab, N1, N2, N3, out, ldo, stream, group,
+                             nullptr, M);
+}
+
+extern "C" int gn_sa_fused_rows(const float *x, int ldx, int C, const float *pos, const int32_t *centre_idx, const int32_t *nbr,
+                                const int32_t *cnt, int M, int K, int self_loops, const int32_t *self_src, const float *w1p,
+                                const float *w2p, const float *w3p, const float *tab, int N1, int N2, int N3, float *out, int ldo,
+                                void *stream, int group, const int32_t *rows, int R) {
+    GN_REQUIRE(rows != nullptr || R == 0, "gn_sa_fused_rows: rows is NULL");
+    return sa_checked_launch(x, ldx, C, pos, centre_idx, nbr, cnt, M, K, self_loops, self_src, w1p, w2p, w3p, tab, N1, N2, N3, out, ldo, stream, group,
+                             rows, R);
+}
+
 extern "C" int gn_sa_fused_scoped(const float *x, int ldx, int C, const float *pos, const int32_t *centre_idx, const int32_t *nbr,
                                   const int32_t *cnt, int M, int K, int self_loops, const int32_t *self_src, const float *w1p,
                                   const float *w2p, const float *w3p, const float *tab, int N1, int N2, int N3, float *out, int ldo,
diff --git a/garmentnets_amd/ops.py b/garmentnets_amd/ops.py
--- a/garmentnets_amd/ops.py
+++ b/garmentnets_amd/ops.py
@@ -82,6 +82,36 @@
     _lib.call("gn_fps_nested_ws", _p(pos), _p(ptr), _p(out_ptr), _p(start_idx), B, int(max_points), _p(idx), _p(gap_out), _p(nested_gap),
               _p(ws), nbytes, _stream())
     return idx
+
+
+def fps_resume_state_bytes(B, max_points):
+    return int(_lib.load().gn_fps_resume_state_bytes(int(B), int(max_points)))
+
+
+def fps_resume(pos, ptr, out_ptr, max_points, idx, steps, state, start_idx=None, gap_out=None):
+    _chk(pos, torch.float32, "pos")
+    _chk(idx, _i32, "idx")
+    _chk(steps, _i32, "steps")
+    B = ptr.numel() - 1
+    if steps.numel() != 2 * B:
+        raise ValueError(f"fps_resume: steps must be int32 [{B}][2]")
+    if gap_out is not None:
+        _chk(gap_out, torch.float32, "gap_out")
+    _lib.call("gn_fps_resume", _p(pos), _p(ptr), _p(out_ptr), _p(start_idx), B, int(max_points), _p(idx), _p(gap_out), _p(steps),
+              _p(_chk(state, torch.uint8, "state")), state.numel(), _stream())
+    return idx
+
+
+def ball_query_rows(pos, ptr, centre_idx, centre_ptr, r, nbr, cnt, rows):
+    M, K = nbr.shape
+    _chk(nbr, _i32, "nbr")
+    _chk(cnt, _i32, "cnt")
+    if centre_idx.numel() != M or cnt.numel() != M:
+        raise ValueError("ball_query_rows: nbr / cnt must be the full tables of centre_idx")
+    r2 = float(np.float32(float(r) * float(r)))
+    _lib.call("gn_ball_query_rows", _p(pos), _p(ptr), _p(centre_idx), _p(centre_ptr), ptr.numel() - 1, M, r2, K, _p(nbr), _p(cnt),
+              _p(_chk(rows, _i32, "rows")), rows.numel(), _stream())
+    return nbr, cnt
 
 
 def ball_query(pos, ptr, centre_idx, centre_ptr, r, K=64):
@@ -158,6 +188,18 @@
     _lib.call("gn_sa_fused_group", _p(x), ldx, pack.cin, _p(_chk(pos, torch.float32, "pos")), _p(centre_idx), _p(nbr), _p(cnt), M, K, 1 if self_loops else 0,
               _p(_chk(self_src, _i32, "self_src") if self_src is not None else None), _p(pack.w1p), _p(pack.w2p), _p(pack.w3p), _p(pack.tab), pack.dims[0], pack.dims[1], pack.dims[2], _p(out), rows_view(out)[1], _stream(),
               int(group))
+    return out
+
+
+def sa_fused_rows(x, pos, centre_idx, nbr, cnt, pack, out, rows, self_loops=True, self_src=None, group=0):
+    M, K = nbr.shape
+    if out.dtype != torch.float32 or tuple(out.shape) != (M, pack.cout):
+        raise ValueError(f"sa_fused_rows: out must be float32 [{M}][{pack.cout}]")
+    ldx = 0 if x is None else rows_view(x)[1]
+    rows_p = _p(_chk(rows, _i32, "rows"))
+    _lib.call("gn_sa_fused_rows", _p(x), ldx, pack.cin, _p(_chk(pos, torch.float32, "pos")), _p(centre_idx), _p(nbr), _p(cnt), M, K, 1 if self_loops else 0,
+              _p(_chk(self_src, _i32, "self_src") if self_src is not None else None), _p(pack.w1p), _p(pack.w2p), _p(pack.w3p), _p(pack.tab), pack.dims[0], pack.dims[1], pack.dims[2], _p(out), rows_view(out)[1], _stream(),
+              int(group), rows_p, rows.numel())
     return out
 
 
diff --git a/include/garmentnets_hip.h b/include/garmentnets_hip.h
--- a/include/garmentnets_hip.h
+++ b/include/garmentnets_hip.h
@@ -30,9 +30,15 @@
 int gn_fps_nested_ws(const float *pos, const int32_t *ptr, const int32_t *out_ptr, const int32_t *start_idx, int B,
                      int max_points_per_example, int32_t *out_idx, float *gap_out, const float *nested_gap, void *ws, size_t ws_bytes,
                      void *stream);
+size_t gn_fps_resume_state_bytes(int B, int max_points_per_example);
+int gn_fps_resume(const float *pos, const int32_t *ptr, const int32_t *out_ptr, const int32_t *start_idx, int B,
+                  int max_points_per_example, int32_t *out_idx, float *gap_out, const int32_t *steps, void *state, size_t state_bytes,
+                  void *stream);
 
 int gn_ball_query(const float *pos, const int32_t *ptr, const int32_t *centre_idx, const int32_t *centre_ptr, int B,
                   int M, float r2, int K, int32_t *nbr, int32_t *cnt, void *stream);
+int gn_ball_query_rows(const float *pos, const int32_t *ptr, const int32_t *centre_idx, const int32_t *centre_ptr, int B,
+                       int M, float r2, int K, int32_t *nbr, int32_t *cnt, const int32_t *rows, int R, void *stream);
 
 int gn_sa_gather(const float *x, int ldx, int C, const float *pos, const int32_t *centre_idx, const int32_t *nbr,
                  int M, int K, int self_loops, float *out, int ldo, int32_t *slot_src, void *stream);
@@ -52,6 +58,9 @@
 int gn_sa_fused_group(const float *x, int ldx, int C, const float *pos, const int32_t *centre_idx, const int32_t *nbr, const int32_t *cnt,
                       int M, int K, int self_loops, const int32_t *self_src, const float *w1p, const float *w2p, const float *w3p,
                       const float *tab, int N1, int N2, int N3, float *out, int ldo, void *stream, int group);
+int gn_sa_fused_rows(const float *x, int ldx, int C, const float *pos, const int32_t *centre_idx, const int32_t *nbr, const int32_t *cnt,
+                     int M, int K, int self_loops, const int32_t *self_src, const float *w1p, const float *w2p, const float *w3p,
+                     const float *tab, int N1, int N2, int N3, float *out, int ldo, void *stream, int group, const int32_t *rows, int R);
 int gn_sa_fused_auto_group(int C, int N1, int N2, int N3, int M);
 
 int gn_global_max_pool(const float *in, int ldi, const int32_t *ptr, int B, int C, float *out, int ldo, void *stream);
```
